# JuliaNeighbors/IVFADC.jl

Hardware: AMD Instinct MI355X
Metric: queries/sec at recall@1 (k=10), SIFT1M-shape d=128 m=8 k=256, 1/2/4/8 GPU (higher is better)
Workload: dtype f32

## Files before the change

include/ivfadc_hip.h:

```cpp
#ifndef IVFADC_HIP_H
#define IVFADC_HIP_H

#include <stddef.h>
#include <stdint.h>

#ifdef __cplusplus
extern "C" {
#endif

typedef struct ivfadc_index ivfadc_t;

typedef enum {
    IVFADC_OK = 0,
    IVFADC_ERR_ASSERT = 1,
    IVFADC_ERR_INVALID = 2,
    IVFADC_ERR_HIP = 3,
    IVFADC_ERR_STATE = 4
} ivfadc_status;

#define IVFADC_ABI_VERSION 4
int ivfadc_abi_version(void);

#define IVFADC_MAX_K 2048
#define IVFADC_MAX_W 2048
// ... 74 lines not shown
int ivfadc_mg_set_gather(ivfadc_mg_t *g, int mode);
int ivfadc_mg_collectives(ivfadc_mg_t *g, int64_t *out);
int ivfadc_mg_append(ivfadc_mg_t *g, int64_t nnew, const float *pts, const uint32_t *ids,
                     int32_t *out_list, uint8_t *out_codes);
int ivfadc_mg_delete_ids(ivfadc_mg_t *g, int64_t ndel, const uint32_t *ids, int64_t *out_removed);
int ivfadc_mg_shift_ids(ivfadc_mg_t *g, int32_t delta);
int ivfadc_mg_search(ivfadc_mg_t *g, int64_t nq, const float *queries, int K, int w,
                     uint32_t *out_ids, float *out_dists, int32_t *out_counts);
void ivfadc_mg_destroy(ivfadc_mg_t *g);

int ivfadc_comm_unique_id(uint8_t *out_id128);
int ivfadc_comm_init(ivfadc_t *h, int nranks, int rank, const uint8_t *id128);
int ivfadc_search_device_allgather(ivfadc_t *h, int64_t nq, const float *d_queries, int K, int w,
                                   int32_t *d_block, int32_t *d_gathered, int slot);
int ivfadc_search_device_allgather_on(ivfadc_t *h, ivfadc_t *searcher, int64_t nq, const float *d_queries, int K, int w,
                                      int32_t *d_block, int32_t *d_gathered, int slot);
int ivfadc_comm_wait(ivfadc_t *h, int64_t *out_collectives);
int ivfadc_comm_destroy(ivfadc_t *h);

int ivfadc_set_list_partition(ivfadc_t *h, int nparts, int part);
int ivfadc_search_device_partial(ivfadc_t *h, int64_t nq, const float *d_queries, int K, int w, uint64_t *d_keys, int32_t *d_counts);
int ivfadc_merge_partials_device(ivfadc_t *h, int64_t nq, int K, int nparts, const uint64_t *d_keys_all, const int32_t *d_counts_all,
                                 uint32_t *d_ids, float *d_dists, int32_t *d_counts);
int64_t ivfadc_listpart_block_words(int64_t nq, int K);
int ivfadc_search_device_listpart(ivfadc_t *h, int64_t nq, const float *d_queries, int K, int w, int32_t *d_block, int32_t *d_gathered,
                                  uint32_t *d_ids, float *d_dists, int32_t *d_counts);

int ivfadc_set_stream(ivfadc_t *h, void *hip_stream);

int ivfadc_ntotal(ivfadc_t *h, int64_t *out_n, int64_t *list_sizes);

int ivfadc_get_lists(ivfadc_t *h, int64_t *offsets, uint8_t *codes, uint32_t *ids);

int ivfadc_get_dims(ivfadc_t *h, int *d, int *kc, int *m, int *ksub);
int ivfadc_get_quantizers(ivfadc_t *h, float *centroids , float *codebooks , uint8_t *code_labels );

int ivfadc_save_index(ivfadc_t *h, const char *path, int index_bits);

int ivfadc_load_index(ivfadc_t **out, int device, const char *path, int *out_index_bits);

int ivfadc_get_rotation(ivfadc_t *h, int *out_rotated, float *out_rot);

typedef struct {
    double   scan_ms;
    double   coarse_ms;
    int64_t  scan_launches;
    int64_t  scanned_points;
    int64_t  queries;
    int32_t  last_qg;
    int32_t  last_chunk;
    int32_t  last_scan_grid;
    int32_t  last_scan_lds;
    int64_t  coarse_fallbacks;
    int32_t  coarse_mfma;
    int32_t  inplace_appends;
    int32_t  last_striped;
    int32_t  coarse_listed;
    int64_t  pruned_points;
    int64_t  lb_survivors;
    int32_t  last_lb;
    int32_t  last_rider;
    double   lb_build_ms;
    int64_t  lb_build_launches;
    int32_t  coarse_prefetched;
    int32_t  last_nf;
    int32_t  last_twolevel;
    int32_t  twolevel_groups;
    int64_t  coarse_visited;
    float    twolevel_probe_fraction;
    int32_t  coarse_f16;
} ivfadc_stats;

int ivfadc_set_profiling(ivfadc_t *h, int on);
int ivfadc_reset_stats(ivfadc_t *h);
int ivfadc_get_stats(ivfadc_t *h, ivfadc_stats *out);

int ivfadc_set_tuning(ivfadc_t *h, int qg, int chunk_points);

int ivfadc_set_coarse_mode(ivfadc_t *h, int mode);

int ivfadc_set_pruning(ivfadc_t *h, int on);

int ivfadc_set_next_queries(ivfadc_t *h, int64_t nq, const float *d_queries, uint64_t token);
int ivfadc_set_query_token(ivfadc_t *h, uint64_t token);

int ivfadc_set_table_mode(ivfadc_t *h, int mode);

int ivfadc_set_u16_tables(ivfadc_t *h, int mode);

int ivfadc_debug_lb_table(ivfadc_t *h, const float *query, int cell, uint8_t *out_table, float *out_consts);

int ivfadc_set_workspace_limit(ivfadc_t *h, uint64_t bytes);

void ivfadc_destroy(ivfadc_t *h);

const char *ivfadc_last_error(void);

#ifdef __cplusplus
}
#endif
#endif
```

ivfadc.jl_amd/_native.py:

```python
import ctypes as C
import os
import subprocess

_HERE = os.path.dirname(os.path.abspath(__file__))
CSRC = os.path.join(_HERE, "csrc")
SO_PATH = os.path.join(CSRC, "libivfadc_hip.so")
SOURCES = [os.path.join(CSRC, "ivfadc_hip.hip"), os.path.join(CSRC, "kernels.hip.h"), os.path.join(CSRC, "train.hip.h"), os.path.join(CSRC, "wave_sort.hip.h"),
           os.path.join(CSRC, "generic.hip.h"), os.path.join(CSRC, "lbscan.hip.h"), os.path.join(CSRC, "nfscan.hip.h"), os.path.join(CSRC, "smallq.hip.h"), os.path.join(CSRC, "twolevel.hip.h"), os.path.join(CSRC, "wg8scan.hip.h"), os.path.join(CSRC, "u16scan.hip.h"),
           os.path.join(os.path.dirname(_HERE), "include", "ivfadc_hip.h")]

HIPCC_FLAGS = ["--offload-arch=gfx950", "-O3", "-ffp-contract=off", "-fno-slp-vectorize", "-fPIC", "-shared", "-std=c++17"]

OK, ERR_ASSERT, ERR_INVALID, ERR_HIP, ERR_STATE = 0, 1, 2, 3, 4


class IVFADCError(RuntimeError):
    def __init__(self, code, msg):
        super().__init__("ivfadc_hip status %d: %s" % (code, msg))
        self.code = code


def needs_build():
    if not os.path.exists(SO_PATH):
        return True
# ... 5 lines not shown
    if not force and not needs_build():
        return SO_PATH
    hipcc = os.environ.get("HIPCC", "/opt/rocm/bin/hipcc")
    cmd = [hipcc] + HIPCC_FLAGS + ["-o", SO_PATH + ".tmp", SOURCES[0]]
    if verbose:
        print(" ".join(cmd))
    subprocess.check_call(cmd, cwd=CSRC)
    os.replace(SO_PATH + ".tmp", SO_PATH)
    return SO_PATH


class Stats(C.Structure):
    _fields_ = [("scan_ms", C.c_double), ("coarse_ms", C.c_double), ("scan_launches", C.c_int64),
                ("scanned_points", C.c_int64), ("queries", C.c_int64), ("last_qg", C.c_int32),
                ("last_chunk", C.c_int32), ("last_scan_grid", C.c_int32), ("last_scan_lds", C.c_int32),
                ("coarse_fallbacks", C.c_int64), ("coarse_mfma", C.c_int32), ("inplace_appends", C.c_int32),
                ("last_striped", C.c_int32), ("coarse_listed", C.c_int32), ("pruned_points", C.c_int64),
                ("lb_survivors", C.c_int64), ("last_lb", C.c_int32), ("last_rider", C.c_int32),
                ("lb_build_ms", C.c_double), ("lb_build_launches", C.c_int64),
                ("coarse_prefetched", C.c_int32), ("last_nf", C.c_int32), ("last_twolevel", C.c_int32), ("twolevel_groups", C.c_int32),
                ("coarse_visited", C.c_int64), ("twolevel_probe_fraction", C.c_float), ("coarse_f16", C.c_int32)]


class HostStats(C.Structure):
    _fields_ = [("stage_in_us", C.c_double), ("enqueue_us", C.c_double), ("wait_us", C.c_double), ("stage_out_us", C.c_double),
                ("calls", C.c_int64), ("batches", C.c_int64), ("queries_direct", C.c_int64), ("results_direct", C.c_int64),
                ("zero_copy", C.c_int64), ("streams_replaced", C.c_int64)]


ABI_VERSION = 4

_lib = None


def lib():
    global _lib
    if _lib is not None:
        return _lib
    if not os.path.exists(SO_PATH):
        raise IVFADCError(ERR_STATE, "libivfadc_hip.so is not built (run __graft_entry__.build()); "
                                     "there is no CPU fallback")
    L = C.CDLL(SO_PATH)
    vp, fp, u8p = C.c_void_p, C.POINTER(C.c_float), C.POINTER(C.c_uint8)
    i32p, u32p, i64p = C.POINTER(C.c_int32), C.POINTER(C.c_uint32), C.POINTER(C.c_int64)
    L.ivfadc_last_error.restype = C.c_char_p
    L.ivfadc_create.argtypes = [C.POINTER(vp), C.c_int, C.c_int, C.c_int, C.c_int, C.c_int, fp, fp, u8p]
    L.ivfadc_set_lists.argtypes = [vp, i64p, u8p, u32p]
    L.ivfadc_create_u16.argtypes = [C.POINTER(vp), C.c_int, C.c_int, C.c_int, C.c_int, C.c_int, fp, fp, vp]
    L.ivfadc_code_bits.argtypes = [vp, C.POINTER(C.c_int)]
    L.ivfadc_set_lists_u16.argtypes = [vp, i64p, vp, u32p]
    L.ivfadc_get_lists_u16.argtypes = [vp, i64p, vp, u32p]
    L.ivfadc_encode_u16.argtypes = [vp, C.c_int64, fp, i32p, vp]
    L.ivfadc_append_u16.argtypes = [vp, C.c_int64, fp, u32p, i32p, vp]
    L.ivfadc_get_quantizers_u16.argtypes = [vp, fp, fp, vp]
    L.ivfadc_train.argtypes = [C.c_int, C.c_int, C.c_int64, fp, C.c_int, C.c_int, C.c_int, C.c_int, C.c_int, C.c_uint64, fp, fp]
    L.ivfadc_train.restype = C.c_int
    L.ivfadc_synth_lists.argtypes = [vp, i64p, C.c_uint64]
    L.ivfadc_encode.argtypes = [vp, C.c_int64, fp, i32p, u8p]
    L.ivfadc_append.argtypes = [vp, C.c_int64, fp, u32p, i32p, u8p]
    L.ivfadc_search.argtypes = [vp, C.c_int64, fp, C.c_int, C.c_int, u32p, fp, i32p]
    L.ivfadc_debug_lb_table.argtypes = [vp, fp, C.c_int, u8p, fp]
    L.ivfadc_get_dims.argtypes = [vp, i32p, i32p, i32p, i32p]
    L.ivfadc_get_quantizers.argtypes = [vp, fp, fp, u8p]
    L.ivfadc_search_device.argtypes = [vp, C.c_int64, vp, C.c_int, C.c_int, vp, vp, vp]
    L.ivfadc_coarse_search.argtypes = [vp, C.c_int64, fp, C.c_int, i32p, fp]
    L.ivfadc_coarse_search_device.argtypes = [vp, C.c_int64, vp, C.c_int, vp, vp]
    L.ivfadc_search_preassigned.argtypes = [vp, C.c_int64, fp, C.c_int, C.c_int, i32p, fp, u32p, fp, i32p]
    L.ivfadc_search_device_preassigned.argtypes = [vp, C.c_int64, vp, C.c_int, C.c_int, vp, vp, vp, vp, vp]
    for name in ("coarse_search", "coarse_search_device", "search_preassigned", "search_device_preassigned"):
        getattr(L, "ivfadc_" + name).restype = C.c_int
    L.ivfadc_sync.argtypes = [vp]
    L.ivfadc_set_stream.argtypes = [vp, vp]
    L.ivfadc_ntotal.argtypes = [vp, i64p, i64p]
    L.ivfadc_get_lists.argtypes = [vp, i64p, u8p, u32p]
    L.ivfadc_set_profiling.argtypes = [vp, C.c_int]
    L.ivfadc_reset_stats.argtypes = [vp]
    L.ivfadc_get_stats.argtypes = [vp, C.POINTER(Stats)]
    L.ivfadc_set_tuning.argtypes = [vp, C.c_int, C.c_int]
    L.ivfadc_set_workspace_limit.argtypes = [vp, C.c_uint64]
    L.ivfadc_set_coarse_mode.argtypes = [vp, C.c_int]
    L.ivfadc_set_pruning.argtypes = [vp, C.c_int]
    L.ivfadc_set_next_queries.argtypes = [vp, C.c_int64, C.c_void_p, C.c_uint64]
    L.ivfadc_set_query_token.argtypes = [vp, C.c_uint64]
    L.ivfadc_search_batches.argtypes = [vp, C.c_int, i64p, fp, C.c_int, C.c_int, u32p, fp, i32p]
    L.ivfadc_set_table_mode.argtypes = [vp, C.c_int]
    L.ivfadc_set_u16_tables.argtypes = [vp, C.c_int]
    L.ivfadc_set_u16_tables.restype = C.c_int
    L.ivfadc_delete_ids.argtypes = [vp, C.c_int64, u32p, i64p]
    L.ivfadc_shift_ids.argtypes = [vp, C.c_int32]
    L.ivfadc_save_index.argtypes = [vp, C.c_char_p, C.c_int]
    L.ivfadc_load_index.argtypes = [C.POINTER(vp), C.c_int, C.c_char_p, C.POINTER(C.c_int)]
    L.ivfadc_get_rotation.argtypes = [vp, C.POINTER(C.c_int), fp]
    L.ivfadc_destroy.argtypes = [vp]
    L.ivfadc_destroy.restype = None
    L.ivfadc_abi_version.argtypes = []
    L.ivfadc_abi_version.restype = C.c_int
    if L.ivfadc_abi_version() != ABI_VERSION:
        raise IVFADCError(ERR_STATE, "libivfadc_hip.so has ABI version %d, this binding was written for %d: rebuild "
                                     "(__graft_entry__.build())" % (L.ivfadc_abi_version(), ABI_VERSION))
    L.ivfadc_host_alloc.argtypes = [C.c_size_t, C.POINTER(vp)]
    L.ivfadc_host_free.argtypes = [vp]
    L.ivfadc_host_register.argtypes = [vp, C.c_size_t]
    L.ivfadc_host_unregister.argtypes = [vp]
    L.ivfadc_get_host_stats.argtypes = [vp, C.POINTER(HostStats)]
    L.ivfadc_reset_host_stats.argtypes = [vp]
    for name in ("host_alloc", "host_free", "host_register", "host_unregister", "get_host_stats", "reset_host_stats"):
        getattr(L, "ivfadc_" + name).restype = C.c_int
    L.ivfadc_mg_create.argtypes = [C.POINTER(vp), C.c_int, i32p, C.c_int, C.c_int, C.c_int, C.c_int, fp, fp, u8p]
    L.ivfadc_mg_set_lists.argtypes = [vp, i64p, u8p, u32p]
    L.ivfadc_mg_append.argtypes = [vp, C.c_int64, fp, u32p, i32p, u8p]
    L.ivfadc_mg_delete_ids.argtypes = [vp, C.c_int64, u32p, i64p]
    L.ivfadc_mg_shift_ids.argtypes = [vp, C.c_int32]
    L.ivfadc_mg_search.argtypes = [vp, C.c_int64, fp, C.c_int, C.c_int, u32p, fp, i32p]
    L.ivfadc_mg_synth_lists.argtypes = [vp, i64p, C.c_uint64]
    L.ivfadc_mg_num_devices.argtypes = [vp]
    L.ivfadc_mg_set_gather.argtypes = [vp, C.c_int]
    L.ivfadc_mg_collectives.argtypes = [vp, i64p]
    L.ivfadc_comm_unique_id.argtypes = [u8p]
    L.ivfadc_comm_init.argtypes = [vp, C.c_int, C.c_int, u8p]
    L.ivfadc_search_device_allgather.argtypes = [vp, C.c_int64, vp, C.c_int, C.c_int, vp, vp, C.c_int]
    L.ivfadc_search_device_allgather_on.argtypes = [vp, vp, C.c_int64, vp, C.c_int, C.c_int, vp, vp, C.c_int]
    L.ivfadc_clone_view.argtypes = [vp, C.POINTER(vp)]
    L.ivfadc_set_list_partition.argtypes = [vp, C.c_int, C.c_int]
    L.ivfadc_search_device_partial.argtypes = [vp, C.c_int64, vp, C.c_int, C.c_int, vp, vp]
    L.ivfadc_merge_partials_device.argtypes = [vp, C.c_int64, C.c_int, C.c_int, vp, vp, vp, vp, vp]
    L.ivfadc_listpart_block_words.argtypes = [C.c_int64, C.c_int]
    L.ivfadc_listpart_block_words.restype = C.c_int64
    L.ivfadc_search_device_listpart.argtypes = [vp, C.c_int64, vp, C.c_int, C.c_int, vp, vp, vp, vp, vp]
    L.ivfadc_comm_wait.argtypes = [vp, i64p]
    L.ivfadc_comm_destroy.argtypes = [vp]
    L.ivfadc_mg_destroy.argtypes = [vp]
    L.ivfadc_mg_destroy.restype = None
    for name in ("mg_create", "mg_set_lists", "mg_append", "mg_search", "mg_delete_ids", "mg_shift_ids", "mg_synth_lists",
                 "mg_num_devices", "mg_set_gather", "mg_collectives", "set_list_partition", "search_device_partial", "merge_partials_device", "search_device_listpart", "comm_unique_id", "comm_init", "search_device_allgather", "search_device_allgather_on", "clone_view", "comm_wait", "comm_destroy"):
        getattr(L, "ivfadc_" + name).restype = C.c_int
    for name in ("create", "set_lists", "synth_lists", "encode", "append", "search", "search_device", "sync", "set_stream",
                 "ntotal", "get_lists", "set_profiling", "reset_stats", "get_stats", "set_tuning", "set_workspace_limit", "set_coarse_mode", "set_pruning", "set_table_mode", "set_next_queries", "set_query_token", "search_batches", "save_index", "load_index", "delete_ids", "shift_ids"):
        getattr(L, "ivfadc_" + name).restype = C.c_int
    _lib = L
    return L


def check(rc):
    if rc == OK:
        return
    msg = lib().ivfadc_last_error().decode("utf-8", "replace")
    if rc == ERR_ASSERT:
        raise AssertionError(msg)
    raise IVFADCError(rc, msg)


def ptr(a, ty):
    return None if a is None else a.ctypes.data_as(C.POINTER(ty))


class PinnedArray:

    def __init__(self, shape, dtype):
        import numpy as np
        self.shape = tuple(int(x) for x in (shape if isinstance(shape, (tuple, list)) else (shape,)))
        self.dtype = np.dtype(dtype)
        n = int(np.prod(self.shape)) if self.shape else 1
        self.nbytes = max(1, n * self.dtype.itemsize)
        p = C.c_void_p()
        check(lib().ivfadc_host_alloc(self.nbytes, C.byref(p)))
        self._p = p
        buf = (C.c_char * self.nbytes).from_address(p.value)
        self.a = np.frombuffer(buf, dtype=self.dtype, count=n).reshape(self.shape)

    def close(self):
        if self._p is not None and self._p.value:
            self.a = None
            lib().ivfadc_host_free(self._p)
            self._p = None

    def __del__(self):
        try:
            self.close()
        except Exception:
            pass


def host_register(a):
    assert a.flags["C_CONTIGUOUS"]
    check(lib().ivfadc_host_register(C.c_void_p(a.ctypes.data), a.nbytes))


def host_unregister(a):
    check(lib().ivfadc_host_unregister(C.c_void_p(a.ctypes.data)))
```

ivfadc.jl_amd/csrc/ivfadc_hip.hip:

```cpp
#include "../../include/ivfadc_hip.h"
#include "kernels.hip.h"
#include "train.hip.h"
#include "generic.hip.h"
#include "u16scan.hip.h"
#include "twolevel.hip.h"

#include <algorithm>
#include <atomic>
#include <chrono>
#include <cmath>
#include <cstdarg>
#include <cstdio>
#include <cstdlib>
#include <cstring>
#include <mutex>
#include <new>
#include <stdexcept>
#include <string>
#include <thread>
#include <vector>

#include <dlfcn.h>
#include <execinfo.h>
#include <fcntl.h>
// ... 248 lines not shown
    bool allow_nf = true;
    DevBuf wg8_tabs, wg8_items;
    int wg8_mode = 0;
    int u16_tables = 0;
    bool u16_wide = false;
    bool wg8_wide = false;
    int part_n = 1, part_i = 0;
    uint64_t *partial_keys = nullptr;
    int64_t partial_nq = -1;
    int partial_w = 0, partial_K = 0;
    DevBuf sq_keys, sq_cnt, sq_arrive, cent_t;
    bool allow_sq = true, sq_inside = false;
    bool allow_lb = true;
    bool force_lb = false;
    DevBuf cent_hi, cent_lo, q_hi, q_lo;
    DevBuf cent_f16, q_f16, q_flags;
    float f16_scale = 0.f;
    bool allow_f16 = true, last_coarse_f16 = false;
    int dp32 = 0;
    bool allow_bf16 = true, last_coarse_bf16 = false;
    bool allow_prune = true;
    bool allow_listed = true, last_listed = false;
    void *comm = nullptr;
    int comm_ranks = 0, comm_rank = 0;
    hipStream_t comm_stream = nullptr;
    hipEvent_t comm_ready = nullptr;
    static constexpr int COMM_SLOTS = 8;
    hipEvent_t comm_done[COMM_SLOTS] = {};
    bool comm_busy[COMM_SLOTS] = {};
    int64_t comm_collectives = 0;
    int64_t comm_seq = 0, comm_slot_seq[COMM_SLOTS] = {}, comm_waited = 0;
    bool allow_filt = true;
    DevBuf tl_centres, tl_off, tl_rad, tl_cent, tl_slot, tl_gdist;
    int tl_G = 0, tl_mode = 0;
    bool dev_entry = false;
    PinnedBuf fb_pin;
    hipEvent_t fb_ev = nullptr;
    bool fb_pending = false;
    int fb_countdown = 0;
    int64_t fb_sp = 0, fb_pp = 0;
    float prune_est = -1.0f;
    RelaxedInt lane_ticket;
    int my_ticket = -1;
    RelaxedInt n_views;
    bool tl_tried = false, tl_use = false;
    float tl_eps = 0.f, tl_probe_fraction = -1.f;
    int64_t visited_base = 0;
    DevBuf gen_a, gen_b, gen_tmp, gen_off, gen_tot;
    int tlist_ldq = 0;
    int tmin_tiles = 0, tmin_tile_w = 0;
    float cmaxn = 0.f;
    bool allow_mfma = true;
    int mfma_min_kc = 2048;
    int64_t n = 0;
    bool have_lists = false;
    bool synthetic = false;
    bool dirty = false;
    int64_t maxlen = 0;
    int64_t inplace_appends = 0;
    DevBuf list_pos, list_len, list_codeoff, codes, ids, app_stage;
    std::vector<int64_t> h_len;
    std::vector<std::vector<uint8_t>> hl_codes;
    std::vector<std::vector<uint32_t>> hl_ids;
    std::vector<int64_t> d_cap, d_pos, d_codeoff;
    int64_t ntotal() const
    {
        int64_t t = 0;
        for (int64_t v : h_len) t += v;
        return t;
    }
    std::vector<uint8_t> h_label_ok;
    bool identity_labels = false;
    bool u16 = false;
    int cb = 0;
    std::vector<uint16_t> lab16;
    std::vector<uint32_t> lab_sorted;
    std::vector<float> rot;

    const float *hint_q = nullptr, *pf_q = nullptr, *avail_q = nullptr;
    int64_t hint_nq = 0, pf_nq = 0, avail_nq = 0;
    uint64_t hint_token = 0, pf_token = 0, cur_token = 0, own_token = 0;
    hipEvent_t hint_ev = nullptr;
    DevBuf cdist2;
    DevBuf pre_list, pre_dc;
    DevBuf q_stage, cdist, probe_list, probe_dc, probe_base, list_cnt, bucket_off, wi_off, cursor, bucket_items, misc,
        qthr, part_keys, part_cnt, out_ids, out_dists, out_counts, assign, enc_codes, pts_stage, dbg;
    PinnedBuf pin_in, pin_out;
    bool hc_out_direct = false;
    hipStream_t copy_stream = nullptr;
    hipStream_t copy_probed_a = nullptr, copy_probed_b = nullptr;
    std::vector<hipEvent_t> ingest_ev;
    ivfadc_host_stats hstats{};
    int64_t carry_queries = 0, carry_scanned = 0, carry_pruned = 0, carry_surv = 0, carry_fallbacks = 0, carry_launches = 0;
    size_t qthr_armed = 0;
    bool list_cnt_armed = false;
    size_t ws_budget = (size_t)8 << 30;

    bool profiling = false;
    int profiling_level = 0;
    struct EvPair { hipEvent_t a, b; int kind; };
    std::vector<EvPair> pending;
    std::vector<EvPair> free_ev;
    ivfadc_stats stats{};
    int64_t scanned_base = 0, fallback_base = 0, pruned_base = 0, surv_base = 0;
    int force_qg = 0, force_chunk = 0;
    bool own_stream = true;
    struct FnCfg { const void *fn; size_t lds; int occ; };
    std::vector<FnCfg> fn_cfg;

    ivfadc_index *view_of = nullptr;
    bool is_view = false, orphan = false;
    uint64_t generation = 0, view_gen = 0;
    std::vector<ivfadc_index *> views;
    ivfadc_index *pipe_view = nullptr;
    hipEvent_t pipe_ev_in = nullptr;
};

struct HandleLock {
    ivfadc_index *h;
    explicit HandleLock(ivfadc_index *x) : h(x)
    {
        if (!h) return;
        if (h->is_view) {
            std::lock_guard<std::recursive_mutex> topo(g_topo_mu);
            h->mu.m.lock();
        } else {
            h->mu.m.lock();
        }
    }
    ~HandleLock() { if (h) h->mu.m.unlock(); }
    HandleLock(const HandleLock &) = delete;
    HandleLock &operator=(const HandleLock &) = delete;
};

namespace {

int wait_stream(ivfadc_index *h)
{
    for (int i = 0; i < 200000; ++i) {
        const hipError_t e = hipStreamQuery(h->stream);
        if (e == hipSuccess) return IVFADC_OK;
        if (e != hipErrorNotReady) return fail(IVFADC_ERR_HIP, "hipStreamQuery failed: %s", hipGetErrorString(e));
        if (i > 20000) break;
    }
    HIP_TRY(hipStreamSynchronize(h->stream));
    return IVFADC_OK;
}

int set_device(ivfadc_index *h)
{
    HIP_TRY(hipSetDevice(h->device));
    return IVFADC_OK;
}

int ev_begin(ivfadc_index *h, int kind, ivfadc_index::EvPair &ep)
{
    if (!h->free_ev.empty()) {
        ep = h->free_ev.back();
        h->free_ev.pop_back();
    } else {
        HIP_TRY(hipEventCreate(&ep.a));
        HIP_TRY(hipEventCreate(&ep.b));
    }
    ep.kind = kind;
    HIP_TRY(hipEventRecord(ep.a, h->stream));
    return IVFADC_OK;
// ... 644 lines not shown
        e->max_lds = lds;
    }
    return IVFADC_OK;
}

int fn_occupancy(ivfadc_index *h, const void *fn, size_t lds, int &occ, bool abs_lds = true, int threads = 256)
{
    TRY(fn_raise_lds(h->device, fn, lds, abs_lds));
    occ = 0;
    for (auto &c : h->fn_cfg)
        if (c.fn == fn && c.lds == lds) occ = c.occ;
    if (occ == 0) {
        HIP_TRY(hipOccupancyMaxActiveBlocksPerMultiprocessor(&occ, fn, threads, lds));
        occ = std::max(1, std::min(occ, 8));
        h->fn_cfg.push_back({fn, lds, occ});
    }
    return IVFADC_OK;
}

int run_twolevel(ivfadc_index *h, const float *d_q, int64_t nb, int w, int *d_probe_list, float *d_probe_dc, u32 *d_probe_base, u32 *d_list_cnt,
                 u64 *d_scanned)
{
    const int G = h->tl_G;
    TRY(h->tl_gdist.ensure((size_t)nb * G * 4));
    ivfadc_index::EvPair ep;
    if (h->profiling) TRY(ev_begin(h, 1, ep));
    launch_coarse_exact(h, d_q, nb, h->tl_centres.as<float>(), G, h->tl_gdist.as<float>(), false);
    HIP_TRY(hipGetLastError());
    TwoLevelView tv;
    tv.gdist = h->tl_gdist.as<float>();
    tv.g_off = h->tl_off.as<u32>();
    tv.g_rad = h->tl_rad.as<float>();
    tv.cent_g = h->tl_cent.as<float>();
    tv.slot_id = h->tl_slot.as<u32>();
    tv.G = G;
    tv.d = h->d;
    tv.eps = h->tl_eps;
    const size_t lds = (size_t)4 * h->d * 4 + 4 * 64 * 8;
    if (lds > (size_t)(48 << 10)) TRY(fn_raise_lds(h->device, (const void *)twolevel_topw_kernel, lds, false));
    hipLaunchKernelGGL(twolevel_topw_kernel, dim3((unsigned)((nb + 3) / 4)), dim3(256), lds, h->stream, d_q, tv, (int)nb, w, h->list_len.as<u32>(),
                       d_probe_list, d_probe_dc, d_probe_base, d_list_cnt, d_scanned, h->part_n, h->part_i);
    HIP_TRY(hipGetLastError());
    if (h->profiling) TRY(ev_end(h, ep));
    return IVFADC_OK;
}

int launch_topw(ivfadc_index *h, const float *d_q, int64_t n, int w, int capw, bool mfma, bool wpq4, int *out_list, float *out_dc, u32 *out_base,
                u32 *lc, u64 *counters, int part_n, int part_i)
{
    const size_t lds = (size_t)4 * capw * 8;
    void (*fn)(const float *, int, int, int, int, const u32 *, int *, float *, u32 *, u32 *, u64 *, const RefineArgs, int, int);
    if (mfma)
        fn = wpq4 ? topw_select_kernel<true, 4, true> : topw_select_kernel<true, 1, true>;
    else if (w <= 64)
        fn = wpq4 ? topw_select_kernel<true, 4, false> : topw_select_kernel<true, 1, false>;
    else
        fn = wpq4 ? topw_select_kernel<false, 4, false> : topw_select_kernel<false, 1, false>;
    const unsigned grid = wpq4 ? (unsigned)n : (unsigned)((n + 3) / 4);
    if (lds > (size_t)(32 << 10)) { int occ_unused = 0; TRY(fn_occupancy(h, (const void *)fn, lds, occ_unused, false)); }
    hipLaunchKernelGGL(fn, dim3(grid), dim3(256), lds, h->stream, h->cdist.as<float>(), (int)n, h->kc, w, capw, h->list_len.as<u32>(), out_list,
                       out_dc, out_base, lc, counters, refine_args(h, d_q), part_n, part_i);
    HIP_TRY(hipGetLastError());
    return IVFADC_OK;
}

LbView lb_view(const ivfadc_index *h)
{
    LbView v;
    v.cb_split = h->lb_split.as<uint4>();
    v.cb_n2 = h->lb_n2.as<float>();
    v.cb_lab = h->lb_lab.as<float>();
    v.cb_maxn = h->lb_maxn.as<float>();
    v.cb_f16 = (h->lb_use_f16 && h->lb_f16.p) ? h->lb_f16.as<uint4>() : (const uint4 *)nullptr;
    v.cb_isc = h->lb_isc.as<float>();
    v.mu = v.cb_f16 ? 1.48e-3f : 9.2e-5f;
    return v;
}

int probe_stage(ivfadc_index *h, const Plan &pl, int64_t nb, const float *d_q, int w, bool single, u32 *lc, const int *pre_list, const float *pre_dc)
{
    const bool pre = pre_list != nullptr;
    u64 *d_scanned = h->misc.as<u64>();
    const bool wpq4 = !pl.lanes && nb * 1 < (int64_t)8 * h->num_cu * 4 && h->kc >= 512 && !(pl.form == ScanForm::QueryMajorLb && !pl.fuse_topw);
    const bool have_rows = single && !pre && !pl.coarse_mfma && !pl.twolevel && h->avail_q == d_q && h->avail_nq == nb && h->cdist2.p != nullptr;
    h->avail_q = nullptr;
    if (pre || pl.twolevel || have_rows) {
        h->tmin_tiles = 0;
        h->last_listed = false;
    }
    if (pre) {
        hipLaunchKernelGGL(probe_ingest_kernel, dim3((unsigned)((nb + 3) / 4)), dim3(256), 0, h->stream, pre_list, pre_dc, (int)nb, h->kc, w,
                           h->list_len.as<u32>(), h->probe_list.as<int>(), h->probe_dc.as<float>(), h->probe_base.as<u32>(), lc, (u32 *)nullptr,
                           d_scanned);
        HIP_TRY(hipGetLastError());
    } else if (pl.twolevel) {
        TRY(run_twolevel(h, d_q, nb, w, h->probe_list.as<int>(), h->probe_dc.as<float>(), h->probe_base.as<u32>(), lc, d_scanned));
    } else if (have_rows) {
        std::swap(h->cdist, h->cdist2);
    } else {
        TRY(run_coarse(h, d_q, nb, pl.coarse_mfma, pl.coarse_mfma && (pl.fuse_topw ? h->m > 16 : !wpq4),
                       !pl.fuse_topw && !wpq4, w));
    }
    if (!pl.fuse_topw && !pl.twolevel && !pre)
        TRY(launch_topw(h, d_q, nb, w, pl.capw, pl.coarse_mfma, wpq4, h->probe_list.as<int>(), h->probe_dc.as<float>(), h->probe_base.as<u32>(), lc,
                        d_scanned, h->part_n, h->part_i));
    h->stats.last_rider = 0;
    h->stats.coarse_prefetched = have_rows ? 1 : 0;
    h->stats.last_twolevel = pl.twolevel ? 1 : 0;
    h->stats.coarse_mfma = pl.coarse_mfma ? 1 : 0;
    h->stats.coarse_f16 = (pl.coarse_mfma && h->last_coarse_f16 && !have_rows) ? 1 : 0;
    h->stats.coarse_listed = h->last_listed ? 1 : 0;
    return IVFADC_OK;
}

int scan_query_major(ivfadc_index *h, const Plan &pl, int64_t nb, const float *d_q, int K, int w, uint32_t *d_ids, float *d_dists, int32_t *d_counts,
                     bool single, bool pre)
{
    const int kc = h->kc;
    const bool lb = pl.form == ScanForm::QueryMajorLb;
    QScanArgs a;
    a.ix = index_view(h);
    a.queries = d_q;
    a.nq = (int)nb; a.w = w; a.K = K; a.cap = pl.cap;
    a.probe_list = h->probe_list.as<int>(); a.probe_dc = h->probe_dc.as<float>(); a.probe_base = h->probe_base.as<u32>();
    a.out_ids = d_ids; a.out_dists = d_dists; a.out_counts = d_counts;
    a.cdist = pl.fuse_topw ? h->cdist.as<float>() : (const float *)nullptr;
    a.scanned_points = h->misc.as<u64>();
    a.approx = pl.coarse_mfma ? 1 : 0;
    a.rf = refine_args(h, d_q);
    a.prune = h->allow_prune ? (pre ? 2 : 1) : 0;
    a.lb = lb_view(h);
    int occ = 0;
    TRY(fn_occupancy(h, pl.fn, pl.lds, occ));
    ivfadc_index::EvPair ep;
    const bool ride = single && !pre && !h->tl_use && h->hint_q != nullptr && h->hint_nq > 0 && !lb && pl.small_k && (h->d & 7) == 0 &&
                      (!h->allow_mfma || kc < h->mfma_min_kc) && (h->hint_nq + 4 * RIDER_QW - 1) / (4 * RIDER_QW) <= 65535 &&
                      (size_t)h->hint_nq * kc * 4 <= h->ws_budget / 4;
    qscan_coarse_fn_t fk = ride ? pick_qscan_coarse(h->m, h->dsub, pl.qg) : nullptr;
    if (fk) {
        TRY(h->cdist2.ensure((size_t)h->hint_nq * kc * 4));
        CoarseNext cn;
        cn.queries = h->hint_q; cn.out = h->cdist2.as<float>(); cn.nq = (int)h->hint_nq; cn.ncx = (kc + 63) / 64;
        const size_t lds = std::max<size_t>(pl.lds, (size_t)64 * 132 * 4);
        TRY(fn_raise_lds(h->device, (const void *)fk, lds, true));
        const unsigned grid = (unsigned)(nb + (int64_t)cn.ncx * ((h->hint_nq + 4 * RIDER_QW - 1) / (4 * RIDER_QW)));
        if (h->hint_ev) {
            HIP_TRY(hipStreamWaitEvent(h->stream, h->hint_ev, 0));
            h->hint_ev = nullptr;
        }
        if (h->profiling) TRY(ev_begin(h, 0, ep));
        hipLaunchKernelGGL(fk, dim3(grid), dim3(256), lds, h->stream, a, cn);
        HIP_TRY(hipGetLastError());
        if (h->profiling) TRY(ev_end(h, ep));
        h->pf_q = h->hint_q;
        h->pf_nq = h->hint_nq;
        h->pf_token = h->hint_token;
        h->stats.last_rider = 1;
    } else {
        if (h->profiling) TRY(ev_begin(h, 0, ep));
        hipLaunchKernelGGL((qscan_fn_t)pl.fn, dim3((unsigned)nb), dim3(pl.threads), pl.lds, h->stream, a);
        HIP_TRY(hipGetLastError());
        if (h->profiling) TRY(ev_end(h, ep));
    }
    h->stats.last_scan_grid = (int)nb;
    if (!lb) TRY(fb_snapshot(h));
    if (h->profiling_level >= 2 && lb && !pl.fuse_topw && pl.qg == 4) {
        void (*bk)(const IndexView, const LbView, const float *, const int *, int, u32 *) =
            (h->m == 48) ? lb_build_only_kernel<48, 16, 4> : lb_build_only_kernel<16, 6, 4>;
        TRY(fn_raise_lds(h->device, (const void *)bk, pl.lds, false));
        TRY(h->dbg.ensure((size_t)nb * 4));
        ivfadc_index::EvPair eb;
        TRY(ev_begin(h, 2, eb));
        hipLaunchKernelGGL(bk, dim3((unsigned)nb), dim3(256), pl.lds, h->stream, a.ix, a.lb, d_q, h->probe_list.as<int>(), w,
                           h->dbg.as<u32>());
        HIP_TRY(hipGetLastError());
        TRY(ev_end(h, eb));
    }
    return IVFADC_OK;
}

template <class... P, class... X>
int launch_list_scan(ivfadc_index *h, const Plan &pl, size_t upper, void (*fn)(const ScanArgs, P...), const ScanArgs &a, X... extra)
{
    int occ = 0;
    TRY(fn_occupancy(h, pl.fn, pl.lds, occ, true, pl.threads));
    const unsigned grid = (unsigned)std::max<size_t>(1, std::min<size_t>(upper, (size_t)h->num_cu * occ));
    ivfadc_index::EvPair ep;
    if (h->profiling) TRY(ev_begin(h, 0, ep));
    hipLaunchKernelGGL(fn, dim3(grid), dim3(pl.threads), pl.lds, h->stream, a, extra...);
    HIP_TRY(hipGetLastError());
    if (h->profiling) TRY(ev_end(h, ep));
    h->stats.last_scan_grid = (int)grid;
    return IVFADC_OK;
}

int scan_list_major(ivfadc_index *h, const Plan &pl, int64_t nb, const float *d_q, int K, int w, uint32_t *d_ids, float *d_dists, int32_t *d_counts,
                    bool direct)
{
    const int kc = h->kc;
    const size_t np = (size_t)nb * w;
    const bool w8 = pl.form == ScanForm::EightWave;
    u32 *d_qhead = (u32 *)((char *)h->misc.p + 4096);
    TRY(h->bucket_items.ensure(np * 4));
    TRY(h->part_keys.ensure(np * pl.maxch * K * 8));
    TRY(h->part_cnt.ensure(np * pl.maxch * 4));
    {
        const size_t before = h->qthr.bytes;
        TRY(h->qthr.ensure((size_t)nb * 8));
        if (h->qthr.bytes != before) h->qthr_armed = 0;
        if (h->qthr_armed < (size_t)nb) {
            const size_t cnt = h->qthr.bytes / 8;
            hipLaunchKernelGGL(fill_u64_kernel, dim3(256), dim3(256), 0, h->stream, h->qthr.as<u64>(), cnt, (u64)KEY_MAX);
            HIP_TRY(hipGetLastError());
            h->qthr_armed = cnt;
        }
    }
    if (!direct) {
        u32 *item_list = nullptr;
        if (w8) {
            TRY(h->wg8_items.ensure(np * (size_t)pl.maxch * 4));
            item_list = h->wg8_items.as<u32>();
        }
        hipLaunchKernelGGL(bucket_scan_kernel, dim3(1), dim3(1024), 0, h->stream, h->list_cnt.as<u32>(), h->list_len.as<u32>(),
                           kc, pl.qg, pl.CH, h->bucket_off.as<u32>(), h->wi_off.as<u32>(), h->cursor.as<u32>(), d_qhead, item_list);
        HIP_TRY(hipGetLastError());
        hipLaunchKernelGGL(bucket_scatter_kernel, dim3((unsigned)((np + 255) / 256)), dim3(256), 0, h->stream,
                           h->probe_list.as<int>(), (int)np, h->bucket_off.as<u32>(), h->cursor.as<u32>(), h->bucket_items.as<u32>(),
                           h->part_n, h->part_i);
        HIP_TRY(hipGetLastError());
    }

    ScanArgs a;
    a.ix = index_view(h);
    a.queries = d_q;
    a.w = w; a.K = K; a.cap = pl.cap;
    a.probe_dc = h->probe_dc.as<float>(); a.probe_base = h->probe_base.as<u32>(); a.list_cnt = h->list_cnt.as<u32>();
    a.bucket_off = h->bucket_off.as<u32>(); a.wi_off = h->wi_off.as<u32>(); a.bucket_items = h->bucket_items.as<u32>();
    a.queue_head = d_qhead;
    a.qthr = h->qthr.as<u64>();
    a.part_keys = h->part_keys.as<u64>(); a.part_cnt = h->part_cnt.as<u32>(); a.maxch = pl.maxch; a.CH = pl.CH;
// ... 94 lines not shown

int check_view_current(ivfadc_index *h)
{
    if (!h->is_view) return IVFADC_OK;
    if (h->orphan || !h->view_of) return fail(IVFADC_ERR_STATE, "the index this view was taken from has been destroyed");
    if (h->view_of->generation != h->view_gen) return fail(IVFADC_ERR_STATE, "the index has changed since this view was taken: take a new one");
    return IVFADC_OK;
}

int check_search_args(ivfadc_index *h, int64_t nq, int K, int &w)
{
    if (!h) return fail(IVFADC_ERR_INVALID, "null handle");
    TRY(check_view_current(h));
    if (K < 1) return fail(IVFADC_ERR_ASSERT, "Number of neighbors must be k >= 1");
    if (w < 1) return fail(IVFADC_ERR_ASSERT, "Number of clusters to search in must be w >= 1");
    if (nq < 0) return fail(IVFADC_ERR_INVALID, "nq < 0");
    if (!h->have_lists && !h->dirty) return fail(IVFADC_ERR_STATE, "no inverted lists set");
    w = std::min(w, h->kc);
    if ((int64_t)nq * K > ((int64_t)1 << 40)) return fail(IVFADC_ERR_INVALID, "nq x K = %lld result slots", (long long)nq * K);
    return IVFADC_OK;
}

int gen_sort(ivfadc_index *h, const u64 *in, u64 *out, int64_t total, int segments, const u32 *d_off)
{
    if (total == 0) return IVFADC_OK;
    size_t tmp = 0;
    HIP_TRY(rocprim::segmented_radix_sort_keys(nullptr, tmp, in, out, (unsigned)total, (unsigned)segments, d_off, d_off + 1, 0, 64,
                                               h->stream));
    TRY(h->gen_tmp.ensure(std::max<size_t>(tmp, 16)));
    HIP_TRY(rocprim::segmented_radix_sort_keys(h->gen_tmp.p, tmp, in, out, (unsigned)total, (unsigned)segments, d_off, d_off + 1, 0, 64,
                                               h->stream));
    return IVFADC_OK;
}

int gen_stage_a(ivfadc_index *h, const float *qa, int64_t na, int w, int *d_pl, float *d_pd, u32 *d_pb, u64 *d_scanned)
{
    const int kc = h->kc;
    TRY(run_coarse(h, qa, na, false));
    const int64_t rk = na * kc;
    TRY(h->gen_a.ensure((size_t)rk * 8));
    TRY(h->gen_b.ensure((size_t)rk * 8));
    hipLaunchKernelGGL(gen_row_keys_kernel, dim3((unsigned)std::min<int64_t>(8192, (rk + 255) / 256)), dim3(256), 0, h->stream,
                       h->cdist.as<float>(), rk, kc, h->gen_a.as<u64>());
    HIP_TRY(hipGetLastError());
    std::vector<u32> off((size_t)na + 1);
    for (int64_t q = 0; q <= na; ++q) off[q] = (u32)(q * kc);
    TRY(h->gen_off.ensure(((size_t)na + 1) * 4));
    TRY(h2d_copy(h->gen_off.p, off.data(), ((size_t)na + 1) * 4, h->stream));
    HIP_TRY(hipStreamSynchronize(h->stream));
    TRY(gen_sort(h, h->gen_a.as<u64>(), h->gen_b.as<u64>(), rk, (int)na, h->gen_off.as<u32>()));
    hipLaunchKernelGGL(gen_probes_kernel, dim3((unsigned)na), dim3(256), 0, h->stream, h->gen_b.as<u64>(), kc, w, h->list_len.as<u32>(),
                       d_pl, d_pd, d_pb, h->gen_tot.as<u32>(), d_scanned);
    HIP_TRY(hipGetLastError());
    return IVFADC_OK;
}

int search_generic(ivfadc_index *h, int64_t nq, const float *d_q, int K, int w, uint32_t *d_ids, float *d_dists, int32_t *d_counts,
                   const int *pre_list = nullptr, const float *pre_dc = nullptr)
{
    const int kc = h->kc;
    const size_t lds = (align_up((size_t)h->d, 4) + (h->u16 ? (size_t)GEN16_TILE : (size_t)h->m * 256)) * 4;
    if (lds > LDS_MAX) return fail(IVFADC_ERR_INVALID, "m=%d needs %zu B of LDS in the generic path (> %zu)", h->m, lds, LDS_MAX);
    void (*dump)(const IndexView, const float *, int, const int *, const float *, const u32 *, const u32 *, u64 *) =
        h->u16 ? gen_dump_u16_kernel : gen_dump_kernel;
    TRY(fn_raise_lds(h->device, (const void *)dump, lds, false));
    TRY(ensure_common_ws(h));
    u64 *d_scanned = h->misc.as<u64>();
    const IndexView ix = index_view(h);
    const u32 *idp = h->synthetic ? (const u32 *)nullptr : h->ids.as<u32>();
    const int64_t per_q = (int64_t)kc * (4 + 16) + (int64_t)w * 12 + 64;
    int64_t nba = std::max<int64_t>(1, (int64_t)(h->ws_budget / (size_t)per_q));
    nba = std::min<int64_t>(std::min<int64_t>(nba, nq), std::min<int64_t>(65535, ((int64_t)1 << 31) / std::max(1, kc)));
    std::vector<u32> tot, off;
    for (int64_t a0 = 0; a0 < nq; a0 += nba) {
        const int64_t na = std::min(nba, nq - a0);
        const float *qa = d_q + (size_t)a0 * h->d;
        const size_t np = (size_t)na * w;
        TRY(h->probe_list.ensure(np * 4));
        TRY(h->probe_dc.ensure(np * 4));
        TRY(h->probe_base.ensure(np * 4));
        TRY(h->gen_tot.ensure((size_t)na * 4));
        if (pre_list) {
            hipLaunchKernelGGL(probe_ingest_kernel, dim3((unsigned)((na + 3) / 4)), dim3(256), 0, h->stream, pre_list + (size_t)a0 * w,
                               pre_dc + (size_t)a0 * w, (int)na, kc, w, h->list_len.as<u32>(), h->probe_list.as<int>(), h->probe_dc.as<float>(),
                               h->probe_base.as<u32>(), (u32 *)nullptr, h->gen_tot.as<u32>(), d_scanned);
            HIP_TRY(hipGetLastError());
        } else {
            TRY(gen_stage_a(h, qa, na, w, h->probe_list.as<int>(), h->probe_dc.as<float>(), h->probe_base.as<u32>(), d_scanned));
        }
        tot.resize((size_t)na);
        TRY(d2h_copy(tot.data(), h->gen_tot.p, (size_t)na * 4, h->stream));
        HIP_TRY(hipStreamSynchronize(h->stream));
        const int64_t cap_keys = std::max<int64_t>(1 << 20, (int64_t)(h->ws_budget / 24));
        for (int64_t g0 = 0; g0 < na;) {
            int64_t g1 = g0, keys = 0;
            while (g1 < na && (g1 == g0 || keys + tot[g1] <= cap_keys) && keys + tot[g1] < ((int64_t)1 << 32)) keys += tot[g1++];
            if (g1 == g0) return fail(IVFADC_ERR_INVALID, "a single query probes %u points: too many for one sort", tot[g0]);
            const int64_t ng = g1 - g0;
            off.resize((size_t)ng + 1);
            off[0] = 0;
            for (int64_t q = 0; q < ng; ++q) off[q + 1] = off[q] + tot[g0 + q];
            TRY(h->gen_a.ensure((size_t)std::max<int64_t>(1, keys) * 8));
            TRY(h->gen_b.ensure((size_t)std::max<int64_t>(1, keys) * 8));
            TRY(h->gen_off.ensure(((size_t)ng + 1) * 4));
            TRY(h2d_copy(h->gen_off.p, off.data(), ((size_t)ng + 1) * 4, h->stream));
            const int *pl = h->probe_list.as<int>() + (size_t)g0 * w;
            const float *pd = h->probe_dc.as<float>() + (size_t)g0 * w;
            const u32 *pb = h->probe_base.as<u32>() + (size_t)g0 * w;
            for (int64_t y0 = 0; y0 < ng; y0 += 32768) {
                const int64_t ny = std::min<int64_t>(32768, ng - y0);
                hipLaunchKernelGGL(dump, dim3((unsigned)w, (unsigned)ny), dim3(256), lds, h->stream, ix,
                                   qa + (size_t)(g0 + y0) * h->d, w, pl + (size_t)y0 * w, pd + (size_t)y0 * w, pb + (size_t)y0 * w,
                                   h->gen_off.as<u32>() + y0, h->gen_a.as<u64>());
                HIP_TRY(hipGetLastError());
            }
            TRY(gen_sort(h, h->gen_a.as<u64>(), h->gen_b.as<u64>(), keys, (int)ng, h->gen_off.as<u32>()));
            hipLaunchKernelGGL(gen_emit_kernel, dim3((unsigned)ng), dim3(256), 0, h->stream, h->gen_b.as<u64>(), h->gen_off.as<u32>(),
                               h->gen_tot.as<u32>() + g0, w, K, pl, pb, h->list_pos.as<int64_t>(), idp, d_ids + (size_t)(a0 + g0) * K,
                               d_dists + (size_t)(a0 + g0) * K, d_counts + a0 + g0);
            HIP_TRY(hipGetLastError());
            HIP_TRY(hipStreamSynchronize(h->stream));
            g0 = g1;
        }
        h->stats.queries += na;
    }
    h->stats.last_qg = -2;
    h->stats.coarse_mfma = 0;
    return IVFADC_OK;
}

int sq_inside_kc(const ivfadc_index *h)
{
    return (h->sq_inside && h->cent_t.p) ? SQ_COARSE_INSIDE : 0;
}

bool sq_eligible(const ivfadc_index *h, int64_t nq, int K, int w)
{
    static const bool off = getenv("IVFADC_NO_SMALLQ") != nullptr;
    if (off || !h->allow_sq || h->force_qg != 0 || h->u16) return false;
    if (K > 64 || w > 64 || nq > 64 || nq * w > 512) return false;
    if ((h->d & 3) != 0) return false;
    const size_t lds = scan_lds_bytes(h, 1, 64, true) + 64 + (h->kc <= sq_inside_kc(h) ? (size_t)h->kc * 4 : 0);
    return lds <= LDS_MAX;
}

int search_small(ivfadc_index *h, int64_t nq, const float *d_q, int K, int w, uint32_t *d_ids, float *d_dists, int32_t *d_counts)
{
    TRY(ensure_common_ws(h));
    const bool inside = h->kc <= sq_inside_kc(h);
    if (!inside) {
        if (h->cent_t.p && nq <= 65535) {
            TRY(h->cdist.ensure((size_t)nq * h->kc * 4));
            ivfadc_index::EvPair ec;
            if (h->profiling) TRY(ev_begin(h, 1, ec));
            void (*ck)(const float4 *, const float *, float *, int, int, int) =
                h->d == 128 ? coarse_lane_kernel<32> : (h->d == 96 ? coarse_lane_kernel<24> : (h->d == 64 ? coarse_lane_kernel<16> : coarse_lane_kernel<0>));
            hipLaunchKernelGGL(ck, dim3((unsigned)((h->kc + 255) / 256), (unsigned)nq), dim3(256), 0, h->stream,
                               h->cent_t.as<float4>(), d_q, h->cdist.as<float>(), (int)nq, h->kc, h->d);
            HIP_TRY(hipGetLastError());
            if (h->profiling) TRY(ev_end(h, ec));
        } else {
            TRY(run_coarse(h, d_q, nq, false));
        }
    }
    const int64_t items = nq * w;
    int nch = (int)std::max<int64_t>(1, std::min<int64_t>((h->maxlen + 4095) / 4096, (2 * (int64_t)h->num_cu) / std::max<int64_t>(1, items)));
    uint32_t CH = (uint32_t)align_up((size_t)std::max<int64_t>(1, (h->maxlen + nch - 1) / nch), 1024);
// ... 124 lines not shown
            any = true;
        }
        if (!any) break;
    }
    mem.erase(std::remove_if(mem.begin(), mem.end(), [](const std::vector<int> &l) { return l.empty(); }), mem.end());
    const int G2 = (int)mem.size();
    std::vector<float> gc((size_t)G2 * d);
    std::vector<u32> off((size_t)G2 + 1, 0);
    for (int g = 0; g < G2; ++g) {
        std::vector<float> c_;
        centre_of(mem[g], c_);
        std::copy(c_.begin(), c_.end(), gc.begin() + (size_t)g * d);
        off[g + 1] = off[g] + (u32)mem[g].size();
    }
    const size_t slots = off[G2];
    std::vector<u32> slot_id(std::max<size_t>(slots, 1), 0xFFFFFFFFu);
    std::vector<float> grouped(std::max<size_t>(slots, 1) * d, 0.0f), rad((size_t)G2, 0.0f);
    for (int g = 0; g < G2; ++g) {
        const u32 ns = off[g + 1] - off[g];
        float *blk = grouped.data() + (size_t)off[g] * d;
        double r2max = 0.0;
        for (u32 sl = 0; sl < ns; ++sl) {
            const int c = mem[g][sl];
            slot_id[off[g] + sl] = (u32)c;
            for (int i = 0; i < d; ++i) blk[((size_t)(i >> 2) * ns + sl) * 4 + (i & 3)] = cent[(size_t)c * d + i];
            r2max = std::max(r2max, dist2(c, &gc[(size_t)g * d]));
        }
        rad[g] = std::nextafter((float)(std::sqrt(r2max) * (1.0 + 1e-6)), INFINITY);
    }
    TRY(h->tl_centres.ensure(gc.size() * 4));
    TRY(h->tl_off.ensure(off.size() * 4));
    TRY(h->tl_rad.ensure(rad.size() * 4));
    TRY(h->tl_cent.ensure(grouped.size() * 4 + 64));
    TRY(h->tl_slot.ensure(slot_id.size() * 4));
    TRY(h2d_copy(h->tl_centres.p, gc.data(), gc.size() * 4, h->stream));
    TRY(h2d_copy(h->tl_off.p, off.data(), off.size() * 4, h->stream));
    TRY(h2d_copy(h->tl_rad.p, rad.data(), rad.size() * 4, h->stream));
    TRY(h2d_copy(h->tl_cent.p, grouped.data(), grouped.size() * 4, h->stream));
    TRY(h2d_copy(h->tl_slot.p, slot_id.data(), slot_id.size() * 4, h->stream));
    G = G2;
    h->tl_G = G;
    h->tl_eps = (float)(d + 16) * 1.1920929e-7f;
    {
        const int64_t ns = std::min<int64_t>(1024, kc);
        const int wp = std::min(32, kc);
        TRY(ensure_common_ws(h));
        DevBuf pl_, pd_, pb_;
        int rc = pl_.ensure((size_t)ns * wp * 4);
        if (rc == IVFADC_OK) rc = pd_.ensure((size_t)ns * wp * 4);
        if (rc == IVFADC_OK) rc = pb_.ensure((size_t)ns * wp * 4);
        u64 before[512], after[512];
        if (rc == IVFADC_OK) {
            HIP_TRY(hipStreamSynchronize(h->stream));
            HIP_TRY(hipMemcpy(before, h->misc.p, sizeof(before), hipMemcpyDeviceToHost));
            const bool prof = h->profiling;
            h->profiling = false;
            rc = run_twolevel(h, h->centroids.as<float>(), ns, wp, pl_.as<int>(), pd_.as<float>(), pb_.as<u32>(), nullptr, h->misc.as<u64>());
            h->profiling = prof;
        }
        if (rc == IVFADC_OK) {
            HIP_TRY(hipStreamSynchronize(h->stream));
            HIP_TRY(hipMemcpy(after, h->misc.p, sizeof(after), hipMemcpyDeviceToHost));
            u64 vis = 0;
            for (int i = 0; i < 64; ++i) vis += after[i * 8 + 3] - before[i * 8 + 3];
            HIP_TRY(h2d_hip(h->misc.p, before, sizeof(before), h->stream));
            h->tl_probe_fraction = (float)((double)vis / ((double)ns * (double)kc));
        }
        pl_.release(); pd_.release(); pb_.release();
        if (rc != IVFADC_OK) return rc;
    }
    h->tl_use = h->tl_mode > 0 || (h->tl_mode == 0 && h->tl_probe_fraction >= 0.f && h->tl_probe_fraction <= TL_AUTO_MAX_FRACTION);
    return IVFADC_OK;
}

struct PreProbes { const int *lists; const float *dcs; };

int search_dev(ivfadc_index *h, int64_t nq, const float *d_q, int K, int w, uint32_t *d_ids, float *d_dists, int32_t *d_counts,
               const PreProbes *pre = nullptr)
{
    HintScope hint_scope{h};
    const bool declared = h->cur_token != 0 && h->cur_token == h->pf_token;
    h->avail_q = declared ? h->pf_q : nullptr;
    h->avail_nq = declared ? h->pf_nq : 0;
    h->pf_q = nullptr; h->pf_nq = 0; h->pf_token = 0; h->cur_token = 0;
    h->stats.coarse_prefetched = 0;
    h->stats.last_rider = 0;
    h->partial_nq = -1;
    TRY(set_device(h));
    if (h->dirty) TRY(upload_lists(h));
    if (nq == 0) return IVFADC_OK;
    if (!pre && !h->tl_tried && !h->is_view && h->tl_mode >= 0 && (h->tl_mode > 0 || h->kc >= TL_AUTO_MIN_KC)) TRY(build_twolevel(h));
    const bool parted = h->part_n > 1;
    const int *prl = pre ? pre->lists : (const int *)nullptr;
    const float *prd = pre ? pre->dcs : (const float *)nullptr;
    if (!parted && !pre && sq_eligible(h, nq, K, w)) return search_small(h, nq, d_q, K, w, d_ids, d_dists, d_counts);
    if (K > IVFADC_MAX_K || w > IVFADC_MAX_W || h->force_qg == -2 || (h->u16 && K > 64 && !h->u16_wide)) {
        if (parted) return fail(IVFADC_ERR_INVALID, "list-partitioned mode reaches K <= %d and w <= %d", IVFADC_MAX_K, IVFADC_MAX_W);
        return search_generic(h, nq, d_q, K, w, d_ids, d_dists, d_counts, prl, prd);
    }
    Plan pl;
    TRY(fb_poll(h));
    TRY(h->u16 ? make_plan_u16(h, nq, K, w, pl, pre != nullptr) : make_plan(h, nq, K, w, pl, pre != nullptr));
    if (!pl.fits) {
        if (parted) return fail(IVFADC_ERR_INVALID, "list-partitioned mode: the selection kernels' LDS need exceeds a CU for this m and K");
        return search_generic(h, nq, d_q, K, w, d_ids, d_dists, d_counts, prl, prd);
    }
    if (parted && pl.nb < nq)
        return fail(IVFADC_ERR_INVALID, "list-partitioned mode: the batch must fit one sub-batch (raise ivfadc_set_workspace_limit or split the batch)");
    for (int64_t b0 = 0; b0 < nq; b0 += pl.nb) {
        const int64_t nb = std::min(pl.nb, nq - b0);
        TRY(search_subbatch(h, pl, nb, d_q + (size_t)b0 * h->d, K, w, d_ids + (size_t)b0 * K, d_dists + (size_t)b0 * K,
                            d_counts + b0, pl.nb >= nq, pre ? prl + (size_t)b0 * w : prl, pre ? prd + (size_t)b0 * w : prd));
    }
    return IVFADC_OK;
}

int coarse_dev(ivfadc_index *h, int64_t nq, const float *d_q, int w, int32_t *d_lists, float *d_dists)
{
    HintScope hint_scope{h};
    h->pf_q = nullptr; h->pf_nq = 0; h->pf_token = 0; h->cur_token = 0;
    h->stats.coarse_prefetched = 0;
    h->stats.last_rider = 0;
    h->partial_nq = -1;
    TRY(set_device(h));
    if (h->dirty) TRY(upload_lists(h));
    if (nq == 0) return IVFADC_OK;
    if (!h->tl_tried && !h->is_view && h->tl_mode >= 0 && (h->tl_mode > 0 || h->kc >= TL_AUTO_MIN_KC)) TRY(build_twolevel(h));
    TRY(ensure_common_ws(h));
    const int kc = h->kc;
    u64 *d_sink = (u64 *)((char *)h->misc.p + MISC_SINK);
    const bool generic = w > IVFADC_MAX_W;
    const CoarseForm cf = coarse_form(h, w, !generic, true);
    const bool twolevel = cf.twolevel, mfma = cf.mfma;
    const size_t per_q = (twolevel ? (size_t)h->tl_G : (size_t)kc) * (generic ? 20 : 4) + (size_t)w * 4 + 64;
    int64_t nb = (int64_t)std::max<size_t>(generic ? 1 : 64, h->ws_budget / per_q);
    nb = std::min<int64_t>(nb, (int64_t)1 << 22);
    if (twolevel) nb = std::min<int64_t>(nb, std::max<int64_t>(1, ((int64_t)1 << 30) / std::max(1, h->tl_G)));
    if (generic) nb = std::min<int64_t>(nb, std::min<int64_t>(65535, ((int64_t)1 << 31) / std::max(1, kc)));
    nb = std::max<int64_t>(1, std::min<int64_t>(nb, nq));
    TRY(h->probe_base.ensure((size_t)nb * w * 4));
    h->stats.last_twolevel = twolevel ? 1 : 0;
    h->stats.coarse_mfma = mfma ? 1 : 0;
    for (int64_t b0 = 0; b0 < nq; b0 += nb) {
        const int64_t n = std::min(nb, nq - b0);
        const float *q = d_q + (size_t)b0 * h->d;
        int *ol = (int *)d_lists + (size_t)b0 * w;
        float *od = d_dists + (size_t)b0 * w;
        if (generic) {
            TRY(h->gen_tot.ensure((size_t)n * 4));
            TRY(gen_stage_a(h, q, n, w, ol, od, h->probe_base.as<u32>(), d_sink));
            continue;
        }
        if (twolevel) {
            TRY(run_twolevel(h, q, n, w, ol, od, h->probe_base.as<u32>(), nullptr, d_sink));
            h->tmin_tiles = 0;
            h->last_listed = false;
            continue;
        }
        const bool wpq4 = n < (int64_t)8 * h->num_cu * 4 && kc >= 512;
        TRY(run_coarse(h, q, n, mfma, mfma && !wpq4, !wpq4, w));
        TRY(launch_topw(h, q, n, w, sel_cap(w), mfma, wpq4, ol, od, h->probe_base.as<u32>(), nullptr, d_sink, 1, 0));
        h->stats.coarse_f16 = (mfma && h->last_coarse_f16) ? 1 : 0;
        h->stats.coarse_listed = h->last_listed ? 1 : 0;
    }
    return IVFADC_OK;
}

int encode_dev(ivfadc_index *h, int64_t n, const float *pts, int32_t *out_list, uint8_t *out_codes)
{
    const int64_t bmax = std::max<int64_t>(256, (int64_t)(((size_t)1 << 30) / ((size_t)h->kc * 4)));
    const size_t lds = align_up((size_t)h->d, 4) * 4 + (size_t)h->m * 8;
    for (int64_t b0 = 0; b0 < n; b0 += bmax) {
        const int64_t nb = std::min(bmax, n - b0);
        TRY(h->pts_stage.ensure((size_t)nb * h->d * 4));
        TRY(h->assign.ensure((size_t)nb * 4));
        TRY(h->enc_codes.ensure((size_t)nb * h->cb));
        TRY(h2d_copy(h->pts_stage.p, pts + (size_t)b0 * h->d, (size_t)nb * h->d * 4, h->stream));
        TRY(run_coarse(h, h->pts_stage.as<float>(), nb, false));
        hipLaunchKernelGGL(argmin_rows_kernel, dim3((unsigned)((nb + 3) / 4)), dim3(256), 0, h->stream, h->cdist.as<float>(), (int)nb,
                           h->kc, h->assign.as<int>());
        HIP_TRY(hipGetLastError());
        if (h->u16)
            hipLaunchKernelGGL(encode_u16_kernel, dim3((unsigned)nb), dim3(256), lds, h->stream, h->pts_stage.as<float>(), h->assign.as<int>(),
                               h->d, h->m, h->ksub, h->dsub, h->centroids.as<float>(), h->codebooks.as<float>(), h->enc_codes.as<uint16_t>());
        else
        hipLaunchKernelGGL(encode_kernel, dim3((unsigned)nb), dim3(256), lds, h->stream, h->pts_stage.as<float>(), h->assign.as<int>(),
                           h->d, h->m, h->ksub, h->dsub, h->centroids.as<float>(), h->codebooks.as<float>(), h->labels.as<uint8_t>(),
                           h->enc_codes.as<uint8_t>());
        HIP_TRY(hipGetLastError());
        TRY(d2h_copy(out_list + b0, h->assign.p, (size_t)nb * 4, h->stream));
        TRY(d2h_copy(out_codes + (size_t)b0 * h->cb, h->enc_codes.p, (size_t)nb * h->cb, h->stream));
        HIP_TRY(hipStreamSynchronize(h->stream));
    }
    return IVFADC_OK;
}

}

namespace {

struct TrainCtx {
    hipStream_t stream = nullptr;
    DevBuf cdist, assign, mind, partial, acc, counts, flag, blockmax;
};

// ... 427 lines not shown
                        }
                    }
                }
            }
            if (rc == IVFADC_OK) rc = h->cent_hi.ensure(hi.size() * 2);
            if (rc == IVFADC_OK) rc = h->cent_lo.ensure(lo.size() * 2);
            if (rc == IVFADC_OK) {
                e = h2d_hip(h->cent_hi.p, hi.data(), hi.size() * 2, h->stream);
                if (e == hipSuccess) e = h2d_hip(h->cent_lo.p, lo.data(), lo.size() * 2, h->stream);
                if (e != hipSuccess) rc = fail(IVFADC_ERR_HIP, "upload failed: %s", hipGetErrorString(e));
            }
        } else {
            h->allow_bf16 = false;
        }
        if (getenv("IVFADC_NO_PRUNE") != nullptr) h->allow_prune = false;
        if (rc == IVFADC_OK) rc = h->cnorm.ensure((size_t)kc * 4);
        if (rc == IVFADC_OK) {
            e = h2d_hip(h->cnorm.p, cn.data(), (size_t)kc * 4, h->stream);
            if (e != hipSuccess) rc = fail(IVFADC_ERR_HIP, "upload failed: %s", hipGetErrorString(e));
        }
        h->allow_filt = getenv("IVFADC_EXACT_TABLES") == nullptr;
        h->allow_mfma = getenv("IVFADC_COARSE_EXACT") == nullptr;
    }
    if (rc != IVFADC_OK) { ivfadc_destroy(h); return rc; }
    h->h_len.assign((size_t)kc, 0);
    h->hl_codes.assign((size_t)kc, {});
    h->hl_ids.assign((size_t)kc, {});
    h->dirty = true;
    *out = h;
    return IVFADC_OK;
}

int ivfadc_create(ivfadc_t **out, int device, int d, int kc, int m, int ksub, const float *centroids, const float *codebooks,
                  const uint8_t *code_labels)
try {
    return create_impl(out, device, d, kc, m, ksub, centroids, codebooks, code_labels, nullptr);
} IVF_CATCH

int ivfadc_create_u16(ivfadc_t **out, int device, int d, int kc, int m, int ksub, const float *centroids, const float *codebooks,
                      const void *code_labels)
try {
    if (!code_labels) {
        if (out) *out = nullptr;
        return fail(IVFADC_ERR_INVALID, "null array");
    }
    return create_impl(out, device, d, kc, m, ksub, centroids, codebooks, nullptr, (const uint16_t *)code_labels);
} IVF_CATCH

int ivfadc_code_bits(ivfadc_t *h, int *bits)
try {
    HandleLock lk_(h);
    if (!h || !bits) return fail(IVFADC_ERR_INVALID, "null argument");
    *bits = h->u16 ? 16 : 8;
    return IVFADC_OK;
} IVF_CATCH

void ivfadc_destroy(ivfadc_t *h)
{
    if (!h) return;
    std::unique_lock<std::recursive_mutex> topo(g_topo_mu);
    h->mu.m.lock();
    h->mu.m.unlock();
    (void)hipSetDevice(h->device);
    if (h->pipe_view) { ivfadc_destroy(h->pipe_view); h->pipe_view = nullptr; }
    if (h->fb_ev) { (void)hipEventSynchronize(h->fb_ev); (void)hipEventDestroy(h->fb_ev); }
    h->fb_pin.release();
    if (h->pipe_ev_in) (void)hipEventDestroy(h->pipe_ev_in);
    if (h->copy_stream) { (void)hipStreamSynchronize(h->copy_stream); (void)hipStreamDestroy(h->copy_stream); }
    for (hipEvent_t e : h->ingest_ev) (void)hipEventDestroy(e);
    for (ivfadc_index *v : h->views) {
        std::lock_guard<std::recursive_mutex> vl(v->mu.m);
        v->orphan = true;
        v->view_of = nullptr;
    }
    if (h->is_view && h->view_of) {
        auto &vs = h->view_of->views;
        vs.erase(std::remove(vs.begin(), vs.end(), h), vs.end());
        h->view_of->n_views.store((int)vs.size());
    }
    if (h->stream) (void)hipStreamSynchronize(h->stream);
    if (h->comm || h->comm_stream) (void)ivfadc_comm_destroy(h);
    for (auto &ep : h->pending) { (void)hipEventDestroy(ep.a); (void)hipEventDestroy(ep.b); }
    for (auto &ep : h->free_ev) { (void)hipEventDestroy(ep.a); (void)hipEventDestroy(ep.b); }
    DevBuf *bufs[] = {&h->lb_f16, &h->lb_isc, &h->cent_f16, &h->q_f16, &h->q_flags, &h->tl_centres, &h->tl_off, &h->tl_rad, &h->tl_cent, &h->tl_slot, &h->tl_gdist, &h->cdist2, &h->pre_list, &h->pre_dc, &h->cent_t, &h->sq_keys, &h->sq_cnt, &h->sq_arrive, &h->lb_split, &h->lb_n2, &h->lb_lab, &h->lb_maxn, &h->nf_n2, &h->nf_lab, &h->wg8_tabs, &h->wg8_items, &h->centroids, &h->codebooks, &h->codebooks_t, &h->codebooks_p, &h->labels, &h->cnorm, &h->tmin, &h->tlist, &h->cent_hi, &h->cent_lo, &h->q_hi, &h->q_lo, &h->gen_a, &h->gen_b, &h->gen_tmp, &h->gen_off, &h->gen_tot, &h->list_pos, &h->list_len, &h->list_codeoff, &h->codes, &h->ids, &h->app_stage, &h->q_stage,
                      &h->cdist, &h->probe_list, &h->probe_dc, &h->probe_base, &h->list_cnt, &h->bucket_off, &h->wi_off, &h->cursor,
                      &h->bucket_items, &h->misc, &h->qthr, &h->part_keys, &h->part_cnt, &h->out_ids, &h->out_dists, &h->out_counts,
                      &h->assign, &h->enc_codes, &h->pts_stage, &h->dbg};
    for (DevBuf *b : bufs) b->release();
    h->pin_in.release();
    h->pin_out.release();
    if (h->stream && h->own_stream) (void)hipStreamDestroy(h->stream);
    delete h;
}

static int streams_serialised(hipStream_t a, hipStream_t b, bool &serial)
{
    serial = false;
    double best = 1e30;
    for (int rep = 0; rep < 2; ++rep) {
        HIP_TRY(hipStreamSynchronize(a));
        HIP_TRY(hipStreamSynchronize(b));
        const auto t0 = std::chrono::steady_clock::now();
        hipLaunchKernelGGL(spin_us_kernel, dim3(1), dim3(64), 0, a, 60u);
        hipLaunchKernelGGL(spin_us_kernel, dim3(1), dim3(64), 0, b, 60u);
        HIP_TRY(hipGetLastError());
        HIP_TRY(hipStreamSynchronize(a));
        HIP_TRY(hipStreamSynchronize(b));
        best = std::min(best, std::chrono::duration<double, std::micro>(std::chrono::steady_clock::now() - t0).count());
    }
    serial = best > 105.0;
    return IVFADC_OK;
}

static int ensure_overlap(const hipStream_t *fixed, int nfixed, hipStream_t *cand, int64_t *replaced)
{
    static const bool off = getenv("IVFADC_NO_STREAM_PROBE") != nullptr;
    if (off) return IVFADC_OK;
    std::vector<hipStream_t> rejected;
    int rc = IVFADC_OK;
    for (int attempt = 0; attempt < 6; ++attempt) {
        bool clash = false;
        for (int i = 0; i < nfixed && !clash && rc == IVFADC_OK; ++i) {
            if (!fixed[i] || fixed[i] == *cand) continue;
            rc = streams_serialised(fixed[i], *cand, clash);
        }
        if (rc != IVFADC_OK || !clash) break;
        hipStream_t next = nullptr;
        if (hipStreamCreateWithFlags(&next, hipStreamNonBlocking) != hipSuccess) { (void)hipGetLastError(); break; }
        rejected.push_back(*cand);
        *cand = next;
        if (replaced) ++*replaced;
    }
    for (hipStream_t s : rejected) (void)hipStreamDestroy(s);
    return rc;
}

static int clone_view(ivfadc_index *src, ivfadc_index **out)
{
    *out = nullptr;
    if (src->is_view) return fail(IVFADC_ERR_STATE, "a view of a view: take it from the index itself");
    TRY(set_device(src));
    if (src->dirty) TRY(upload_lists(src));
    if (!src->have_lists) return fail(IVFADC_ERR_STATE, "no inverted lists set");
    HIP_TRY(hipStreamSynchronize(src->stream));
    std::vector<std::vector<uint8_t>> keep_codes;
    std::vector<std::vector<uint32_t>> keep_ids;
    keep_codes.swap(src->hl_codes);
    keep_ids.swap(src->hl_ids);
    ivfadc_index *v = nullptr;
    try { v = new ivfadc_index(*src); } catch (...) { keep_codes.swap(src->hl_codes); keep_ids.swap(src->hl_ids); throw; }
    keep_codes.swap(src->hl_codes);
    keep_ids.swap(src->hl_ids);
    DevBuf *shared[] = {&v->lb_f16, &v->lb_isc, &v->cent_f16, &v->tl_centres, &v->tl_off, &v->tl_rad, &v->tl_cent, &v->tl_slot, &v->centroids, &v->codebooks, &v->codebooks_t, &v->codebooks_p, &v->labels, &v->cnorm, &v->lb_split, &v->lb_n2, &v->lb_lab,
                        &v->lb_maxn, &v->nf_n2, &v->nf_lab, &v->cent_t, &v->cent_hi, &v->cent_lo, &v->list_pos, &v->list_len, &v->list_codeoff,
                        &v->codes, &v->ids};
    for (DevBuf *b : shared) b->alias();
    DevBuf *scratch[] = {&v->wg8_tabs, &v->wg8_items, &v->q_f16, &v->q_flags, &v->tl_gdist, &v->cdist2, &v->pre_list, &v->pre_dc, &v->sq_keys, &v->sq_cnt, &v->sq_arrive, &v->tmin, &v->tlist, &v->q_hi, &v->q_lo, &v->gen_a, &v->gen_b, &v->gen_tmp,
                         &v->gen_off, &v->gen_tot, &v->app_stage, &v->q_stage, &v->cdist, &v->probe_list, &v->probe_dc, &v->probe_base, &v->list_cnt,
                         &v->bucket_off, &v->wi_off, &v->cursor, &v->bucket_items, &v->misc, &v->qthr, &v->part_keys, &v->part_cnt, &v->out_ids,
                         &v->out_dists, &v->out_counts, &v->assign, &v->enc_codes, &v->pts_stage, &v->dbg};
    for (DevBuf *b : scratch) b->forget();
    v->pin_in.forget();
    v->pin_out.forget();
    v->pending.clear();
    v->free_ev.clear();
    v->views.clear();
    v->n_views.store(0);
    v->my_ticket = -1;
    v->fb_pin.forget();
    v->fb_ev = nullptr;
    v->fb_pending = false;
    v->fb_countdown = 0;
    v->fb_sp = v->fb_pp = 0;
    v->pipe_view = nullptr;
    v->pipe_ev_in = nullptr;
    v->copy_stream = nullptr;
    v->copy_probed_a = v->copy_probed_b = nullptr;
    v->ingest_ev.clear();
    v->hstats = ivfadc_host_stats{};
    v->carry_queries = v->carry_scanned = v->carry_pruned = v->carry_surv = v->carry_fallbacks = v->carry_launches = 0;
    v->comm = nullptr;
    v->comm_stream = nullptr;
    v->comm_ready = nullptr;
    for (int i = 0; i < ivfadc_index::COMM_SLOTS; ++i) { v->comm_done[i] = nullptr; v->comm_busy[i] = false; }
    v->comm_ranks = 0;
    v->comm_rank = 0;
    v->comm_collectives = 0;
    v->comm_seq = 0;
    v->comm_waited = 0;
    for (int i = 0; i < ivfadc_index::COMM_SLOTS; ++i) v->comm_slot_seq[i] = 0;
    v->hint_ev = nullptr;
    v->hint_q = v->pf_q = v->avail_q = nullptr;
    v->hint_nq = v->pf_nq = v->avail_nq = 0;
    v->hint_token = v->pf_token = v->cur_token = 0;
    v->partial_keys = nullptr;
    v->partial_nq = -1;
    v->qthr_armed = 0;
    v->list_cnt_armed = false;
    v->profiling = false;
    v->profiling_level = 0;
    v->stats = ivfadc_stats{};
    v->scanned_base = v->fallback_base = v->pruned_base = v->surv_base = 0;
    v->visited_base = 0;
    v->inplace_appends = 0;
    v->stream = nullptr;
    v->own_stream = true;
    v->is_view = true;
    v->view_of = src;
    v->view_gen = src->generation;
    const hipError_t e = hipStreamCreateWithFlags(&v->stream, hipStreamNonBlocking);
    if (e != hipSuccess) {
        delete v;
        return fail(IVFADC_ERR_HIP, "hipStreamCreateWithFlags failed: %s", hipGetErrorString(e));
    }
    {
        const hipStream_t fixed[1] = {src->stream};
        const int rc = ensure_overlap(fixed, 1, &v->stream, &src->hstats.streams_replaced);
        if (rc != IVFADC_OK) { (void)hipStreamDestroy(v->stream); delete v; return rc; }
    }
    {
        std::lock_guard<std::recursive_mutex> topo(g_topo_mu);
        src->views.push_back(v);
        src->n_views.fetch_add(1);
    }
    *out = v;
    return IVFADC_OK;
}

static void copy_search_config(ivfadc_index *dst, const ivfadc_index *src)
{
    dst->wg8_mode = src->wg8_mode; dst->wg8_wide = src->wg8_wide; dst->u16_wide = src->u16_wide; dst->u16_tables = src->u16_tables;
    dst->allow_nf = src->allow_nf; dst->allow_sq = src->allow_sq; dst->sq_inside = src->sq_inside; dst->allow_lb = src->allow_lb;
    dst->force_lb = src->force_lb; dst->allow_bf16 = src->allow_bf16; dst->allow_f16 = src->allow_f16; dst->lb_use_f16 = src->lb_use_f16; dst->allow_prune = src->allow_prune; dst->allow_listed = src->allow_listed;
    dst->allow_filt = src->allow_filt; dst->allow_mfma = src->allow_mfma; dst->mfma_min_kc = src->mfma_min_kc; dst->ws_budget = src->ws_budget;
    dst->force_qg = src->force_qg; dst->force_chunk = src->force_chunk;
    dst->part_n = src->part_n; dst->part_i = src->part_i;
    dst->tl_use = src->tl_use && dst->tl_cent.p != nullptr; dst->tl_mode = src->tl_mode;
}

int ivfadc_clone_view(ivfadc_t *h, ivfadc_t **out)
try {
    HandleLock lk_(h);
    if (!h || !out) return fail(IVFADC_ERR_INVALID, "null argument");
    return clone_view(h, out);
} IVF_CATCH

static int check_width(ivfadc_index *h, bool want_u16, const char *what)
{
    if (h->u16 && !want_u16) return fail(IVFADC_ERR_STATE, "%s: this index has UInt16 codes; use %s_u16", what, what);
    if (!h->u16 && want_u16) return fail(IVFADC_ERR_STATE, "%s: this index has UInt8 codes; use the entry without _u16", what);
    return IVFADC_OK;
}

static int check_offsets(ivfadc_index *h, const int64_t *offsets, const void *codes, const uint32_t *ids)
{
    const int kc = h->kc;
    if (offsets[0] != 0) return fail(IVFADC_ERR_INVALID, "offsets[0] must be 0");
    for (int l = 0; l < kc; ++l)
        if (offsets[l + 1] < offsets[l]) return fail(IVFADC_ERR_INVALID, "offsets must be non-decreasing (list %d)", l);
    const int64_t n = offsets[kc];
    if (n > (int64_t)0xFFFFFFFFll) return fail(IVFADC_ERR_ASSERT, "index capacity of UInt32 ids exceeded");
    if (n > 0 && (!codes || !ids)) return fail(IVFADC_ERR_INVALID, "null codes/ids");
    return IVFADC_OK;
}

static int set_lists_mirror(ivfadc_t *h, const int64_t *offsets, const uint8_t *codes, const uint32_t *ids, const char *what)
{
    const int kc = h->kc, cb = h->cb;
    TRY(set_device(h));
    MutationScope ms;
    TRY(ms.begin(h, what));
    for (int l = 0; l < kc; ++l) {
        const int64_t a = offsets[l], b = offsets[l + 1];
        h->h_len[l] = b - a;
        h->hl_codes[l].assign(codes + (size_t)a * cb, codes + (size_t)b * cb);
        h->hl_ids[l].assign(ids + a, ids + b);
    }
    return upload_lists(h);
}

static int labels_to_indices(const ivfadc_index *h, int64_t n, const uint16_t *lab, std::vector<uint8_t> &out)
{
    const int m = h->m;
    out.resize((size_t)n * h->cb);
    uint16_t *dst = (uint16_t *)out.data();
    for (int64_t p = 0; p < n; ++p)
        for (int i = 0; i < m; ++i) {
            const uint16_t v = lab[(size_t)p * m + i];
            const int32_t c = h->identity_labels ? (v < h->ksub ? (int32_t)v : -1) : find_label16(h->lab_sorted, h->ksub, i, v);
            if (c < 0) return fail(IVFADC_ERR_INVALID, "code %d of point %lld is not a label of codebook %d", (int)v, (long long)p, i);
            dst[(size_t)p * m + i] = (uint16_t)c;
        }
    return IVFADC_OK;
}

static void indices_to_labels(const ivfadc_index *h, int64_t n, uint16_t *codes)
{
    if (h->identity_labels) return;
    const int m = h->m, ksub = h->ksub;
    for (int64_t p = 0; p < n; ++p)
        for (int i = 0; i < m; ++i) codes[(size_t)p * m + i] = h->lab16[(size_t)i * ksub + codes[(size_t)p * m + i]];
}

int ivfadc_set_lists_u16(ivfadc_t *h, const int64_t *offsets, const void *codes, const uint32_t *ids)
try {
    HandleLock lk_(h);
    if (!h || !offsets) return fail(IVFADC_ERR_INVALID, "null argument");
    TRY(check_width(h, true, "ivfadc_set_lists"));
    TRY(check_mutable(h, "ivfadc_set_lists_u16"));
    TRY(check_offsets(h, offsets, codes, ids));
    std::vector<uint8_t> idx;
    TRY(labels_to_indices(h, offsets[h->kc], (const uint16_t *)codes, idx));
    return set_lists_mirror(h, offsets, idx.data(), ids, "ivfadc_set_lists_u16");
} IVF_CATCH

int ivfadc_set_lists(ivfadc_t *h, const int64_t *offsets, const uint8_t *codes, const uint32_t *ids)
try {
// ... 1478 lines not shown
        for (int i = 0; i < 64; ++i) pp += shards[i * 8 + 1];
        for (int i = 0; i < 64; ++i) sv += shards[i * 8 + 2];
        for (int i = 0; i < 64; ++i) vis += shards[i * 8 + 3];
        HIP_TRY(hipMemcpy(&h->fallback_base, (char *)h->misc.p + 4096 + 64, 8, hipMemcpyDeviceToHost));
    }
    h->scanned_base = sp;
    h->pruned_base = pp;
    h->surv_base = sv;
    h->visited_base = vis;
    const int qg = h->stats.last_qg, ch = h->stats.last_chunk, gr = h->stats.last_scan_grid, lds = h->stats.last_scan_lds;
    const int cm = h->stats.coarse_mfma, ls = h->stats.last_striped, cl = h->stats.coarse_listed, llb = h->stats.last_lb, lnf = h->stats.last_nf;
    const int ltl = h->stats.last_twolevel, lf16 = h->stats.coarse_f16;
    h->stats = ivfadc_stats{};
    h->stats.last_twolevel = ltl;
    h->stats.coarse_f16 = lf16;
    h->stats.last_lb = llb;
    h->stats.last_nf = lnf;
    h->stats.coarse_mfma = cm;
    h->stats.last_striped = ls;
    h->stats.coarse_listed = cl;
    h->stats.last_qg = qg; h->stats.last_chunk = ch; h->stats.last_scan_grid = gr; h->stats.last_scan_lds = lds;
    h->carry_queries = h->carry_scanned = h->carry_pruned = h->carry_surv = h->carry_fallbacks = h->carry_launches = 0;
    if (h->pipe_view) TRY(ivfadc_reset_stats(h->pipe_view));
    return IVFADC_OK;
} IVF_CATCH

int ivfadc_get_stats(ivfadc_t *h, ivfadc_stats *out)
try {
    HandleLock lk_(h);
    if (!h || !out) return fail(IVFADC_ERR_INVALID, "null argument");
    TRY(set_device(h));
    TRY(ev_fold(h));
    HIP_TRY(hipStreamSynchronize(h->stream));
    int64_t sp = 0, pp = 0, sv = 0, vis = 0;
    if (h->misc.p) {
        int64_t shards[512];
        HIP_TRY(hipMemcpy(shards, h->misc.p, sizeof(shards), hipMemcpyDeviceToHost));
        for (int i = 0; i < 64; ++i) sp += shards[i * 8];
        for (int i = 0; i < 64; ++i) pp += shards[i * 8 + 1];
        for (int i = 0; i < 64; ++i) sv += shards[i * 8 + 2];
        for (int i = 0; i < 64; ++i) vis += shards[i * 8 + 3];
        int64_t fb = 0;
        HIP_TRY(hipMemcpy(&fb, (char *)h->misc.p + 4096 + 64, 8, hipMemcpyDeviceToHost));
        h->stats.coarse_fallbacks = fb - h->fallback_base;
    }
    h->stats.scanned_points = sp - h->scanned_base;
    h->stats.pruned_points = pp - h->pruned_base;
    h->stats.lb_survivors = sv - h->surv_base;
    h->stats.coarse_visited = vis - h->visited_base;
    h->stats.twolevel_groups = h->tl_use ? h->tl_G : 0;
    h->stats.twolevel_probe_fraction = h->tl_probe_fraction;
    h->stats.inplace_appends = (int32_t)std::min<int64_t>(h->inplace_appends, 0x7fffffff);
    *out = h->stats;
    out->queries += h->carry_queries;
    out->scanned_points += h->carry_scanned;
    out->pruned_points += h->carry_pruned;
    out->lb_survivors += h->carry_surv;
    out->coarse_fallbacks += h->carry_fallbacks;
    out->scan_launches += h->carry_launches;
    if (h->pipe_view) {
        ivfadc_stats v;
        TRY(ivfadc_get_stats(h->pipe_view, &v));
        out->queries += v.queries;
        out->scanned_points += v.scanned_points;
        out->pruned_points += v.pruned_points;
        out->lb_survivors += v.lb_survivors;
        out->coarse_fallbacks += v.coarse_fallbacks;
        out->scan_launches += v.scan_launches;
        out->coarse_visited += v.coarse_visited;
    }
    return IVFADC_OK;
} IVF_CATCH

int ivfadc_train(int device, int d, int64_t n, const float *data, int kc, int k, int m, int coarse_maxiter, int quant_maxiter,
                 uint64_t seed, float *out_centroids, float *out_codebooks)
try {
    return train_impl(device, d, n, data, kc, k, m, coarse_maxiter, quant_maxiter, seed, out_centroids, out_codebooks);
} IVF_CATCH

int ivfadc_set_coarse_mode(ivfadc_t *h, int mode)
try {
    HandleLock lk_(h);
    if (!h) return fail(IVFADC_ERR_INVALID, "null handle");
    if (mode < 0 || mode > 8) return fail(IVFADC_ERR_INVALID, "mode must be 0 ... 8");
    h->allow_f16 = mode != 8 && mode != 3;
    h->tl_mode = mode == 6 ? 1 : (mode == 7 ? -1 : 0);
    if (h->tl_tried) h->tl_use = h->tl_G > 0 && (h->tl_mode > 0 || (h->tl_mode == 0 && h->tl_probe_fraction >= 0.f && h->tl_probe_fraction <= 0.02f));
    if (h->tl_mode > 0 && h->tl_G == 0) h->tl_tried = false;
    h->sq_inside = mode == 5;
    h->allow_mfma = (mode != 1) && getenv("IVFADC_COARSE_EXACT") == nullptr;
    h->mfma_min_kc = (mode == 2) ? 128 : 2048;
    h->allow_bf16 = mode != 3 && h->cent_hi.p != nullptr;
    h->allow_listed = mode != 4;
    return IVFADC_OK;
} IVF_CATCH

int ivfadc_set_pruning(ivfadc_t *h, int on)
try {
    HandleLock lk_(h);
    if (!h) return fail(IVFADC_ERR_INVALID, "null handle");
    h->allow_prune = on != 0 && getenv("IVFADC_NO_PRUNE") == nullptr;
    return IVFADC_OK;
} IVF_CATCH

int ivfadc_set_next_queries(ivfadc_t *h, int64_t nq, const float *d_queries, uint64_t token)
try {
    HandleLock lk_(h);
    if (!h) return fail(IVFADC_ERR_INVALID, "null handle");
    if (nq < 0) return fail(IVFADC_ERR_INVALID, "nq < 0");
    h->hint_q = (nq > 0 && token != 0) ? d_queries : nullptr;
    h->hint_nq = h->hint_q ? nq : 0;
    h->hint_token = h->hint_q ? token : 0;
    return IVFADC_OK;
} IVF_CATCH

int ivfadc_set_query_token(ivfadc_t *h, uint64_t token)
try {
    HandleLock lk_(h);
    if (!h) return fail(IVFADC_ERR_INVALID, "null handle");
    h->cur_token = token;
    return IVFADC_OK;
} IVF_CATCH

int ivfadc_set_table_mode(ivfadc_t *h, int mode)
try {
    HandleLock lk_(h);
    if (!h) return fail(IVFADC_ERR_INVALID, "null handle");
    if (mode < 0 || mode > 10) return fail(IVFADC_ERR_INVALID, "mode must be 0 ... 10");
    h->allow_filt = mode != 1 && getenv("IVFADC_EXACT_TABLES") == nullptr;
    h->force_lb = mode == 2 || mode == 4;
    h->lb_use_f16 = mode != 3 && mode != 4;
    h->wg8_mode = mode == 5 ? -1 : (mode == 6 || mode == 8 ? 1 : (mode == 7 || mode == 9 ? 2 : 0));
    h->wg8_wide = mode == 8 || mode == 9;
    h->u16_wide = mode == 10;
    return IVFADC_OK;
} IVF_CATCH

int ivfadc_set_u16_tables(ivfadc_t *h, int mode)
try {
    HandleLock lk_(h);
    if (!h) return fail(IVFADC_ERR_INVALID, "null handle");
    if (mode < 0 || mode > 2) return fail(IVFADC_ERR_INVALID, "mode must be 0 ... 2");
    h->u16_tables = mode;
    return IVFADC_OK;
} IVF_CATCH

int ivfadc_debug_lb_table(ivfadc_t *h, const float *query, int cell, uint8_t *out_table, float *out_consts)
try {
    HandleLock lk_(h);
    if (!h || !query || !out_table || !out_consts) return fail(IVFADC_ERR_INVALID, "null argument");
    if (cell < 0 || cell >= h->kc) return fail(IVFADC_ERR_INVALID, "cell out of range");
    if (h->u16) return fail(IVFADC_ERR_STATE, "ivfadc_debug_lb_table: this index has UInt16 codes (no 8-bit lower-bound tables)");
    if (!h->lb_split.p || !lb_shape(h->m, h->dsub)) return fail(IVFADC_ERR_STATE, "no matrix-core table kernels for m=%d dsub=%d", h->m, h->dsub);
    TRY(set_device(h));
    const int m = h->m;
    DevBuf dq, dt, df;
    int rc = dq.ensure((size_t)h->d * 4);
    if (rc == IVFADC_OK) rc = dt.ensure((size_t)m * 256);
    if (rc == IVFADC_OK) rc = df.ensure((size_t)(3 + 2 * m) * 4);
    if (rc == IVFADC_OK) {
        hipError_t e = hipMemcpyAsync(dq.p, query, (size_t)h->d * 4, hipMemcpyHostToDevice, h->stream);
        if (e == hipSuccess) {
            const size_t lds = lb_lds_bytes(m, h->dsub, 1);
            void (*dk)(const IndexView, const LbView, const float *, int, unsigned char *, float *) =
                (m == 48) ? lb_debug_kernel<48, 16> : lb_debug_kernel<16, 6>;
            rc = fn_raise_lds(h->device, (const void *)dk, lds, false);
            if (rc == IVFADC_OK) {
                hipLaunchKernelGGL(dk, dim3(1), dim3(256), lds, h->stream, index_view(h), lb_view(h), dq.as<float>(), cell, dt.as<unsigned char>(),
                                   df.as<float>());
                e = hipGetLastError();
            }
        }
        if (e == hipSuccess) e = hipMemcpyAsync(out_table, dt.p, (size_t)m * 256, hipMemcpyDeviceToHost, h->stream);
        if (e == hipSuccess) e = hipMemcpyAsync(out_consts, df.p, (size_t)(3 + 2 * m) * 4, hipMemcpyDeviceToHost, h->stream);
        if (e == hipSuccess) e = hipStreamSynchronize(h->stream);
        if (e != hipSuccess && rc == IVFADC_OK) rc = fail(IVFADC_ERR_HIP, "debug table: %s", hipGetErrorString(e));
    }
    dq.release(); dt.release(); df.release();
    return rc;
} IVF_CATCH

int ivfadc_set_workspace_limit(ivfadc_t *h, uint64_t bytes)
try {
    HandleLock lk_(h);
    if (!h) return fail(IVFADC_ERR_INVALID, "null handle");
    h->ws_budget = (size_t)std::max<uint64_t>(bytes, 1 << 20);
    return IVFADC_OK;
} IVF_CATCH

int ivfadc_set_tuning(ivfadc_t *h, int qg, int chunk_points)
try {
    HandleLock lk_(h);
    if (!h) return fail(IVFADC_ERR_INVALID, "null handle");
    if (!(qg == 0 || qg == -1 || qg == -2 || qg == -3 || qg == 1 || qg == 2 || qg == 4 || qg == 8))
        return fail(IVFADC_ERR_INVALID, "qg must be 0, -1, -2, -3, 1, 2, 4 or 8");
// ... 243 lines not shown
```

ivfadc.jl_amd/csrc/kernels.hip.h:

```cpp
#pragma once
#include <hip/hip_runtime.h>
#include <stdint.h>
#include <type_traits>
#include "wave_sort.hip.h"

typedef unsigned long long u64;
typedef unsigned int u32;
typedef float v2f __attribute__((ext_vector_type(2)));
typedef float v4f __attribute__((ext_vector_type(4)));

#define KEY_MAX 0xFFFFFFFFFFFFFFFFull


namespace ivf {

static __device__ __forceinline__ int lane_id()
{
    return (int)__builtin_amdgcn_mbcnt_hi(~0u, __builtin_amdgcn_mbcnt_lo(~0u, 0u));
}

static __device__ __forceinline__ void wave_sync()
{
    __builtin_amdgcn_fence(__ATOMIC_RELEASE, "wavefront");
    __builtin_amdgcn_wave_barrier();
// ... 1336 lines not shown
        __syncthreads();
    }
    u64 *buf = sbuf + (size_t)wv * cap;
    const int Ksel = APPROX ? approx_pool(w) : w;
    WSel<SMALL> sel;
    sel.init(KEY_MAX, buf, cap, Ksel);
    const float *row = cdist + (size_t)q * kc;
    bool tiled = false, listed = false;
    int cnt = 0;
    if constexpr (APPROX && SMALL && WPQ == 1) {
        if (rf.tlist) {
            listed = true;
            const WSel<true> ex = select_listed(q, w, rf, lane, (int *)buf);
            cnt = ex.finish(w, lane);
            wave_sync();
            ex.store(buf, cnt, lane);
        } else if (rf.tmin)
            tiled = select_row_tiled(sel, row, rf.tmin + (size_t)q * rf.ntiles, rf.ntiles, rf.tile_w, kc, Ksel, lane, (int *)buf);
    }
    if (!listed) {
    bool shortrow = false;
    if constexpr (WPQ == 4 && SMALL) {
        if (Ksel <= SHORT_ROW_MAXK && kc <= 2048 && (kc & 3) == 0) {
            __shared__ u64 s_wb[4];
            __shared__ u32 s_cc;
            shortrow = select_row_short<APPROX>(sel, row, kc, Ksel, wv, lane, (int)threadIdx.x, sbuf, s_wb, &s_cc);
            if (shortrow && wv != 0) return;
        }
    }
    if (!tiled && !shortrow) select_row<APPROX, WPQ>(sel, row, kc, Ksel, wv, lane, WPQ == 4 ? &s_thr : (u64 *)nullptr);
    cnt = sel.finish(Ksel, lane);
    if (shortrow) wave_sync();
    sel.store(buf, cnt, lane);
    if (WPQ == 4 && !shortrow) {
        if (lane == 0) s_cnt[wv] = cnt;
        __syncthreads();
        if (wv != 0) return;
        merge_waves(sel, sbuf, (size_t)cap, s_cnt, 1, Ksel, KEY_MAX, 0, lane);
        cnt = sel.finish(Ksel, lane);
        sel.store(buf, cnt, lane);
    }
    if constexpr (APPROX && SMALL) {
        const WSel<true> ex = refine_probes(sel, cnt, w, q, rf, lane);
        cnt = ex.finish(w, lane);
        wave_sync();
        ex.store(buf, cnt, lane);
    }
    }
    wave_sync();
    u32 running = 0, mine_total = 0;
    for (int j0 = 0; j0 < cnt; j0 += 64) {
        const int j = j0 + lane;
        u32 len = 0;
        int l = 0;
        float dd = 0.0f;
        if (j < cnt) {
            const u64 key = buf[j];
            l = (int)(u32)key;
            dd = __uint_as_float((u32)(key >> 32));
            len = list_len[l];
        }
        const bool mine = nparts <= 1 || (l % nparts) == part;
        u32 incl = len, minc = mine ? len : 0u;
#pragma unroll
        for (int off = 1; off < 64; off <<= 1) {
            const u32 v = __shfl_up(incl, off);
            if (lane >= off) incl += v;
        }
#pragma unroll
        for (int off = 32; off > 0; off >>= 1) minc += __shfl_xor(minc, off);
        if (j < cnt) {
            const size_t o = (size_t)q * w + j;
            probe_list[o] = l;
            probe_dc[o] = dd;
            probe_base[o] = running + incl - len;
            if (list_cnt && mine) atomicAdd(&list_cnt[l], 1u);
        }
        running += __shfl(incl, 63);
        mine_total += minc;
    }
    if (lane == 0) atomicAdd(scanned_points + (size_t)(q & 63) * 8, (u64)mine_total);
}

__global__ __launch_bounds__(256) void probe_ingest_kernel(const int *__restrict__ src_list, const float *__restrict__ src_dc, int nq, int kc,
                                                           int w, const u32 *__restrict__ list_len, int *__restrict__ probe_list,
                                                           float *__restrict__ probe_dc, u32 *__restrict__ probe_base,
                                                           u32 *__restrict__ list_cnt, u32 *__restrict__ totals,
                                                           u64 *__restrict__ scanned_points)
{
    const int lane = threadIdx.x & 63, wv = threadIdx.x >> 6;
    const int q = blockIdx.x * 4 + wv;
    if (q >= nq) return;
    u32 running = 0;
    for (int j0 = 0; j0 < w; j0 += 64) {
        const int j = j0 + lane;
        const size_t o = (size_t)q * w + j;
        u32 len = 0;
        int l = 0;
        float dd = 0.0f;
        if (j < w) {
            l = min(max(src_list[o], 0), kc - 1);
            dd = src_dc[o];
            if (__float_as_uint(dd) > 0x7F7FFFFFu) dd = 0.0f;
            len = list_len[l];
        }
        u32 incl = len;
#pragma unroll
        for (int off = 1; off < 64; off <<= 1) {
            const u32 v = __shfl_up(incl, off);
            if (lane >= off) incl += v;
        }
        if (j < w) {
            probe_list[o] = l;
            probe_dc[o] = dd;
            probe_base[o] = running + incl - len;
            if (list_cnt) atomicAdd(&list_cnt[l], 1u);
        }
        running += __shfl(incl, 63);
    }
    if (lane == 0) {
        if (totals) totals[q] = running;
        atomicAdd(scanned_points + (size_t)(q & 63) * 8, (u64)running);
    }
}

__global__ __launch_bounds__(1024) void bucket_scan_kernel(const u32 *__restrict__ list_cnt, const u32 *__restrict__ list_len,
                                                           int kc, int QG, u32 CH, u32 *__restrict__ bucket_off,
                                                           u32 *__restrict__ wi_off, u32 *__restrict__ cursor,
                                                           u32 *__restrict__ queue_head, u32 *__restrict__ item_list = nullptr)
{
    __shared__ u32 sa[1024], sb[1024];
    const int tid = threadIdx.x;
    const int per = (kc + 1023) / 1024;
    const int l0 = tid * per, l1 = min(kc, l0 + per);
    u32 suma = 0, sumb = 0;
    for (int l = l0; l < l1; ++l) {
        const u32 cnt = list_cnt[l];
        const u32 len = list_len[l];
        const u32 ng = (cnt + QG - 1) / QG;
        const u32 nch = (len + CH - 1) / CH;
        suma += cnt;
        sumb += ng * nch;
    }
    sa[tid] = suma;
    sb[tid] = sumb;
    __syncthreads();
    for (int off = 1; off < 1024; off <<= 1) {
        u32 va = 0, vb = 0;
        if (tid >= off) { va = sa[tid - off]; vb = sb[tid - off]; }
        __syncthreads();
        sa[tid] += va;
        sb[tid] += vb;
        __syncthreads();
    }
    u32 runa = sa[tid] - suma, runb = sb[tid] - sumb;
    for (int l = l0; l < l1; ++l) {
        const u32 cnt = list_cnt[l];
        const u32 len = list_len[l];
        const u32 ng = (cnt + QG - 1) / QG;
        const u32 nch = (len + CH - 1) / CH;
        bucket_off[l] = runa;
        wi_off[l] = runb;
        cursor[l] = 0;
        if (item_list)
            for (u32 i = 0; i < ng * nch; ++i) item_list[runb + i] = (u32)l;
        runa += cnt;
        runb += ng * nch;
    }
    if (tid == 1023) { bucket_off[kc] = sa[1023]; wi_off[kc] = sb[1023]; queue_head[0] = 0; }
}

__global__ __launch_bounds__(256) void bucket_scatter_kernel(const int *__restrict__ probe_list, int nprobe,
                                                             const u32 *__restrict__ bucket_off, u32 *__restrict__ cursor,
                                                             u32 *__restrict__ bucket_items, int nparts, int part)
{
    const int p = blockIdx.x * 256 + threadIdx.x;
    if (p >= nprobe) return;
    const int l = probe_list[p];
    if (nparts > 1 && (l % nparts) != part) return;
    const u32 pos = bucket_off[l] + atomicAdd(&cursor[l], 1u);
    bucket_items[pos] = (u32)p;
}

struct IndexView {
    const float *centroids;
// ... 1152 lines not shown
                if (pred) key = part_keys[slot * K + i];
            }
            pred = pred && key < sel.thr();
            sel.push(pred, key, K, lane);
        }
    } else
    for (int j = 0; j < w; ++j) {
        const size_t pi = (size_t)q * w + j;
        const int l = probe_list[pi];
        if (nparts > 1 && (l % nparts) != part) continue;
        const u32 len = list_len[l];
        const int nch = (int)((len + CH - 1) / CH);
        const int tot = nch * K;
        for (int e0 = 0; e0 < tot; e0 += 64) {
            const int e = e0 + lane;
            bool pred = e < tot;
            u64 key = KEY_MAX;
            if (pred) {
                const int c = e / K, i = e - c * K;
                const size_t slot = pi * maxch + c;
                pred = (u32)i < part_cnt[slot];
                if (pred) key = part_keys[slot * K + i];
            }
            pred = pred && key < sel.thr();
            sel.push(pred, key, K, lane);
        }
    }
    const int cnt = sel.finish(K, lane);
    if (out_keys) sel.for_each(cnt, lane, [&](int i, u64 key) { out_keys[(size_t)q * K + i] = key; });
    else sel.for_each(cnt, lane, [&](int i, u64 key) {
        emit_result(key, i, q, w, K, probe_list + (size_t)q * w, probe_base + (size_t)q * w, list_pos, ids, out_ids, out_dists);
    });
    if (lane == 0) {
        out_counts[q] = cnt;
        qthr[q] = KEY_MAX;
    }
}

template <bool SMALL>
__global__ __launch_bounds__(256) void partial_merge_kernel(int nq, int w, int K, int cap, int nranks, const u64 *__restrict__ keys,
                                                            size_t rank_stride_u64, const int *__restrict__ counts, size_t rank_stride_i32,
                                                            const int *__restrict__ probe_list, const u32 *__restrict__ probe_base,
                                                            const int64_t *__restrict__ list_pos, const u32 *__restrict__ ids,
                                                            u32 *__restrict__ out_ids, float *__restrict__ out_dists, int *__restrict__ out_counts)
{
    extern __shared__ __attribute__((aligned(16))) unsigned char smem_raw[];
    u64 *sbuf = (u64 *)smem_raw;
    const int lane = threadIdx.x & 63, wv = threadIdx.x >> 6;
    const int q = blockIdx.x * 4 + wv;
    if (q >= nq) return;
    WSel<SMALL> sel;
    sel.init(KEY_MAX, sbuf + (size_t)wv * cap, cap, K);
    for (int r = 0; r < nranks; ++r) {
        const int c = counts[(size_t)r * rank_stride_i32 + q];
        sel_absorb(sel, keys + (size_t)r * rank_stride_u64 + (size_t)q * K, c < K ? c : K, K, lane);
    }
    const int cnt = sel.finish(K, lane);
    sel.for_each(cnt, lane, [&](int i, u64 key) {
        emit_result(key, i, q, w, K, probe_list + (size_t)q * w, probe_base + (size_t)q * w, list_pos, ids, out_ids, out_dists);
    });
    if (lane == 0) out_counts[q] = cnt;
}

#include "lbscan.hip.h"
#include "nfscan.hip.h"
#include "wg8scan.hip.h"

struct QScanArgs {
    IndexView ix;
    LbView lb;
    const float *queries;
    int nq, w, K, cap;
    const int *probe_list;
    const float *probe_dc;
    const u32 *probe_base;
    u32 *out_ids;
    float *out_dists;
    int *out_counts;
    int prune;
    const float *cdist;
    u64 *scanned_points;
    int approx;
    RefineArgs rf;
};

template <int M, int DS, int PG, bool SMALL, bool LB = false>
static __device__ __forceinline__ void qscan_body(const QScanArgs &a, unsigned char *smem_raw, const int q)
{
    const IndexView &ix = a.ix;
    const int tid = threadIdx.x, lane = tid & 63, wv = tid >> 6;
    const int m = (M > 0) ? M : ix.m;
    const int K = a.K, cap = a.cap, w = a.w;
    static_assert(!LB || (SMALL && M > 0 && DS > 0), "LB rounds: compile-time shape, register selectors");
    LdsCarve L = carve_lds<PG, SMALL, 1>(smem_raw, m, ix.d, cap);
    int stage_floats = (m < 2 ? 2 : m) * 256 * PG;
    if constexpr (LB) {
        using C = LbCfg<M, DS, PG>;
        stage_floats = (int)(C::TAB_BYTES / 4u);
        L.tab = (float *)smem_raw;
        L.resid = nullptr;
        L.selbuf = nullptr;
        L.xch = (u64 *)smem_raw;
        L.xcap = 64;
        L.scnt = (int *)(smem_raw + C::END);
        L.swi = (u32 *)(L.scnt + 4 * PG);
        L.sthr = (u64 *)(L.swi + 4);
    }

    WSel<SMALL> sel[1];
    sel[0].init(KEY_MAX, SMALL ? nullptr : L.selbuf + (size_t)wv * cap, cap, K);
    if (tid == 0) arm_bound<1>(L.sthr, 0, KEY_MAX);

    const int *prow_list = a.probe_list + (size_t)q * w;
    const float *prow_dc = a.probe_dc + (size_t)q * w;
    const u32 *prow_base = a.probe_base + (size_t)q * w;
    const bool cached = w <= 32;
    const int PW = cached ? 32 : 64;
    int *s_list = (int *)(L.sthr + STHR_WORDS * PG);
    float *s_dc = (float *)(s_list + PW);
    u32 *s_base = (u32 *)(s_dc + PW);
    u32 *s_len = s_base + PW;
    u32 *s_coff = s_len + PW;
    if (a.cdist) {
        const int Ksel = a.approx ? approx_pool(w) : w;
        WSel<true> ws;
        ws.init(KEY_MAX, nullptr, 64, Ksel);
        const float *row = a.cdist + (size_t)q * ix.kc;
        __syncthreads();
        bool have = false;
        if constexpr (LB && M > 16) {
            if (Ksel <= SHORT_ROW_MAXK && ix.kc > 2048 && ix.kc <= 8192 && (ix.kc & 3) == 0) {
                u64 *wbound = (u64 *)(s_list + 160);
                u32 *ccnt = (u32 *)(s_list + 168);
                if (ix.kc <= 4096)
                    have = a.approx ? select_row_short<true, 4>(ws, row, ix.kc, Ksel, wv, lane, tid, L.xch, wbound, ccnt)
                                    : select_row_short<false, 4>(ws, row, ix.kc, Ksel, wv, lane, tid, L.xch, wbound, ccnt);
                else
                    have = a.approx ? select_row_short<true, 8>(ws, row, ix.kc, Ksel, wv, lane, tid, L.xch, wbound, ccnt)
                                    : select_row_short<false, 8>(ws, row, ix.kc, Ksel, wv, lane, tid, L.xch, wbound, ccnt);
            }
        }
        if (!have && Ksel <= SHORT_ROW_MAXK && ix.kc <= 2048 && (ix.kc & 3) == 0) {
            u64 *wbound = (u64 *)(s_list + 160);
            u32 *ccnt = (u32 *)(s_list + 168);
            have = a.approx ? select_row_short<true>(ws, row, ix.kc, Ksel, wv, lane, tid, L.xch, wbound, ccnt)
                            : select_row_short<false>(ws, row, ix.kc, Ksel, wv, lane, tid, L.xch, wbound, ccnt);
        }
        if constexpr (M > 16) {
        if (!have && a.approx && a.rf.tmin != nullptr) {
            int *flag = s_list + 170;
            if (wv == 0) {
                const bool ok = select_row_tiled(ws, row, a.rf.tmin + (size_t)q * a.rf.ntiles, a.rf.ntiles, a.rf.tile_w, ix.kc, Ksel, lane,
                                                 (int *)L.xch);
                if (lane == 0) *flag = ok ? 1 : 0;
            }
            __syncthreads();
            have = *flag != 0;
        }
        }
        if (!have) {
            if (a.approx) select_row<true, 4>(ws, row, ix.kc, Ksel, wv, lane, L.sthr);
            else select_row<false, 4>(ws, row, ix.kc, Ksel, wv, lane, L.sthr);
            const int wc = ws.finish(Ksel, lane);
            ws.store(L.xch + (size_t)wv * 64, wc, lane);
            if (lane == 0) L.scnt[wv] = wc;
            __syncthreads();
        }
        int fc = 0;
        if (wv == 0) {
            if (lane == 0) arm_bound<1>(L.sthr, 0, KEY_MAX);
            if (!have) merge_waves(ws, L.xch, (size_t)64, L.scnt, 1, Ksel, KEY_MAX, 0, lane);
            fc = ws.finish(Ksel, lane);
        }
        if (a.approx) {
            ws = refine_probes_wg<(M > 16)>(ws, fc, w, q, a.rf, wv, lane, tid, L.tab, stage_floats, s_list);
            if (wv == 0) fc = ws.finish(w, lane);
        }
        if (wv == 0) {
            u32 len = 0;
            int l = 0;
            if (lane < fc) {
                l = (int)(u32)ws.top;
                len = ix.list_len[l];
            }
            u32 incl = len;
#pragma unroll
            for (int off = 1; off < 64; off <<= 1) {
                const u32 v = __shfl_up(incl, off);
                if (lane >= off) incl += v;
            }
            if (lane < fc) {
                s_list[lane] = l;
                s_dc[lane] = __uint_as_float((u32)(ws.top >> 32));
                s_base[lane] = incl - len;
                if (cached) {
                    s_len[lane] = len;
                    s_coff[lane] = (u32)(ix.list_codeoff[l] >> 8);
                }
            }
            const u32 total = __shfl(incl, 63);
            if (lane == 0) atomicAdd(a.scanned_points + (size_t)(q & 63) * 8, (u64)total);
        }
        __syncthreads();
        prow_list = s_list;
        prow_dc = s_dc;
        prow_base = s_base;
    } else if (cached) {
        if (tid < w) {
            const int l = prow_list[tid];
            s_list[tid] = l;
            s_dc[tid] = prow_dc[tid];
            s_base[tid] = prow_base[tid];
            s_len[tid] = ix.list_len[l];
            s_coff[tid] = (u32)(ix.list_codeoff[l] >> 8);
        }
        __syncthreads();
        prow_list = s_list;
        prow_dc = s_dc;
        prow_base = s_base;
    }
    if constexpr (LB) {
        lb_rounds<M, DS, PG>(ix, a.lb, a.queries, smem_raw, q, w, K, a.prune, a.scanned_points, sel[0], L.sthr, s_list, s_dc, s_base, s_len, s_coff, wv,
                             lane, tid);
    } else {
    constexpr int RU = (M > 0 && M * DS * PG <= 256) ? 1 : 2;
    constexpr bool can_pipe = M == 0 || M * DS * PG <= 256 * RU;
    const bool pipe = can_pipe && cached && ix.d * PG <= 256 * RU;
    float rq[RU], rc[RU];
    auto resid_fetch = [&](int j0) {
#pragma unroll
        for (int u = 0; u < RU; ++u) {
            const int e = tid + u * 256;
            rq[u] = 0.0f;
            rc[u] = 0.0f;
            if (e < ix.d * PG) {
                const int i = e / PG, sl = e - i * PG;
                const int pj = (j0 + sl) < w ? j0 + sl : j0;
                rq[u] = a.queries[(size_t)q * ix.d + i];
                rc[u] = ix.centroids[(size_t)prow_list[pj] * ix.d + i];
            }
        }
    };
    auto resid_store = [&]() {
#pragma unroll
        for (int u = 0; u < RU; ++u) {
            const int e = tid + u * 256;
            if (e < ix.d * PG) L.resid[e] = rq[u] - rc[u];
        }
    };
    if (pipe) {
        resid_fetch(0);
        resid_store();
    }
    int np = PG;
    for (int j0 = 0; j0 < w; j0 += np) {
        np = PG;
        int li[PG], qi[PG];
        u32 len[PG], sb[PG];
        float dcv[PG];
        const uint8_t *cb[PG];
#pragma unroll
        for (int s = 0; s < PG; ++s) {
            const bool ok = (j0 + s) < w;
            const int pj = ok ? j0 + s : j0;
            li[s] = prow_list[pj];
            qi[s] = q;
            dcv[s] = prow_dc[pj];
            sb[s] = prow_base[pj];
            if (cached) {
                len[s] = ok ? s_len[pj] : 0u;
                cb[s] = ix.codes + ((size_t)s_coff[pj] << 8);
            } else {
                len[s] = ok ? ix.list_len[li[s]] : 0u;
                cb[s] = ix.codes + ix.list_codeoff[li[s]];
            }
        }
        CodeRegs<M, ppl_of<M, 1>()> cr[PG];
#pragma unroll
        for (int s = 0; s < PG; ++s) scan_prefetch(cr[s], cb[s], 0u, len[s], wv, lane);
        __syncthreads();
        if (a.prune) {
            const u32 thi = (u32)(readfirstlane64(L.sthr[0]) >> 32);
            if (__float_as_uint(dcv[0]) > thi) {
                if (a.prune == 1) {
                    if (tid == 0) {
                        u64 skipped = 0;
                        for (int pj = j0; pj < w; ++pj) skipped += cached ? s_len[pj] : ix.list_len[prow_list[pj]];
                        atomicAdd(a.scanned_points + (size_t)(q & 63) * 8 + 1, skipped);
                    }
// ... 14 lines not shown
                for (int s = 0; s < PG; ++s) none = none && len[s] == 0;
                if (none) {
                    if (pipe && (j0 + np) < w) {
                        resid_fetch(j0 + np);
                        resid_store();
                    }
                    continue;
                }
            }
            if constexpr (PG == 2 && SMALL) {
                if (j0 == 0 && w > 1 && len[1] != 0 && dcv[1] > 2.0f * dcv[0]) {
                    len[1] = 0;
                    np = 1;
                }
            }
        }
        const int ns = (PG == 2 && len[1 % PG] == 0) ? 1 : PG;
        constexpr bool PKB = M == 48 && DS == 16 && PG == 1;
        const bool pkb = PKB && ix.codebooks_p != nullptr;
        if (!pipe) {
            if (pkb) {
                for (int i = tid; i < ix.d; i += 256) {
                    const int ii = i / DS, t = i - ii * DS;
                    L.resid[((ii >> 1) * DS + t) * 2 + (ii & 1)] = a.queries[(size_t)q * ix.d + i] - ix.centroids[(size_t)li[0] * ix.d + i];
                }
            } else {
                build_residuals<PG>(ix, a.queries, qi, li, L.resid, tid);
            }
            __syncthreads();
        }
        if constexpr (M == 48 && DS == 16) {
            if (pkb) build_tables_pk<DS>(ix, m, L.resid, L.tab, tid);
            else build_tables_deep<PG, DS, 4>(ix, m, L.resid, L.tab, tid);
        } else {
            if constexpr (PG == 2 && DS > 0) {
                if (ns == 1) build_tables_t<PG, DS, TAB_SEP, 0, true>(ix, m, L.resid, L.tab, tid);
                else build_tables_t<PG, DS, TAB_SEP>(ix, m, L.resid, L.tab, tid);
            } else build_tables_t<PG, DS, TAB_SEP>(ix, m, L.resid, L.tab, tid);
        }
        __syncthreads();
        const bool more = pipe && (j0 + np) < w;
        if (more) resid_fetch(j0 + np);
        __builtin_amdgcn_s_setprio(3);
        if constexpr (PG == 2 && M > 0 && M <= 16 && SMALL) {
            scan_pair<M>(0u, (u32)M * 1024u, cb[0], cb[1], len[0], len[1], dcv[0], dcv[1], sb[0], sb[1], sel, K, wv, lane, cr[0], cr[1],
                         L.sthr);
        } else {
#pragma unroll
            for (int s = 0; s < PG; ++s) {
                if (len[s] == 0) continue;
                const float dc1[1] = {dcv[s]};
                const u32 sb1[1] = {sb[s]};
                scan_range<M, 1>(L.tab + (size_t)s * m * 256, (u32)s * (u32)m * 1024u, cb[s], ix.cs, m, 0u, len[s], dc1, sb1, 1, sel, K, wv,
                                 lane, cr[s], L.sthr);
            }
        }
        __builtin_amdgcn_s_setprio(0);
        if (more) resid_store();
    }
    }
    const int mycnt = sel[0].finish(K, lane);
    __syncthreads();
    sel[0].store(L.xch + (size_t)wv * L.xcap, mycnt, lane);
    if (lane == 0) L.scnt[wv] = mycnt;
    __syncthreads();
    if (wv == 0) {
        merge_waves(sel[0], L.xch, (size_t)L.xcap, L.scnt, 1, K, KEY_MAX, 0, lane);
        const int fc = sel[0].finish(K, lane);
        sel[0].for_each(fc, lane, [&](int i, u64 key) {
            emit_result(key, i, q, w, K, prow_list, prow_base, ix.list_pos, ix.ids, a.out_ids, a.out_dists);
        });
        if (lane == 0) a.out_counts[q] = fc;
    }
}

template <int M, int DS, int PG, bool SMALL, bool LB = false>
__global__ __launch_bounds__(256, LB ? (M <= 16 ? 3 : (PG >= 4 ? 2 : (PG == 3 ? 3 : 4))) : 1) void qscan_kernel(const QScanArgs a)
{
    extern __shared__ __attribute__((aligned(16))) unsigned char smem_raw[];
    qscan_body<M, DS, PG, SMALL, LB>(a, smem_raw, (int)blockIdx.x);
}

constexpr int RIDER_QW = 4;
struct CoarseNext {
    const float *queries;
    float *out;
    int nq, ncx;
};
template <int M, int DS, int PG>
__global__ __launch_bounds__(256) void qscan_coarse_kernel(const QScanArgs a, const CoarseNext cn)
{
    extern __shared__ __attribute__((aligned(16))) unsigned char smem_raw[];
    if ((int)blockIdx.x < a.nq) {
        qscan_body<M, DS, PG, true, false>(a, smem_raw, (int)blockIdx.x);
    } else {
        const int t = (int)blockIdx.x - a.nq;
        coarse_sgpr_tile<RIDER_QW>(cn.queries, a.ix.centroids, cn.out, cn.nq, a.ix.kc, a.ix.d, t % cn.ncx, t / cn.ncx, (float *)smem_raw);
    }
}

#include "smallq.hip.h"

__global__ __launch_bounds__(256) void encode_kernel(const float *__restrict__ pts, const int *__restrict__ assign, int d, int m,
                                                     int ksub, int dsub, const float *__restrict__ centroids,
                                                     const float *__restrict__ codebooks, const uint8_t *__restrict__ labels,
                                                     uint8_t *__restrict__ out_codes)
{
    extern __shared__ __attribute__((aligned(16))) unsigned char smem_raw[];
    float *resid = (float *)smem_raw;
    u64 *best = (u64 *)(resid + (((size_t)d + 3) & ~(size_t)3));
    const int p = blockIdx.x, tid = threadIdx.x;
    const int l = assign[p];
    for (int i = tid; i < d; i += 256) resid[i] = pts[(size_t)p * d + i] - centroids[(size_t)l * d + i];
    for (int i = tid; i < m; i += 256) best[i] = KEY_MAX;
    __syncthreads();
    for (int e = tid; e < m * 256; e += 256) {
        const int ii = e >> 8, c = e & 255;
        u64 key = KEY_MAX;
        if (c < ksub) {
            const float *cw = codebooks + ((size_t)ii * ksub + c) * dsub;
            const float *rr = resid + (size_t)ii * dsub;
            float sum = 0.0f;
            for (int t = 0; t < dsub; ++t) {
                const float df = cw[t] - rr[t];
                sum = sum + df * df;
            }
            key = make_key(sum, (u32)c);
        }
#pragma unroll
        for (int off = 32; off > 0; off >>= 1) {
            const u64 o = __shfl_xor(key, off);
            key = o < key ? o : key;
        }
        if ((tid & 63) == 0) atomicMin(&best[ii], key);
    }
    __syncthreads();
    for (int i = tid; i < m; i += 256) out_codes[(size_t)p * m + i] = labels[i * ksub + (int)(u32)best[i]];
}

__global__ __launch_bounds__(256) void argmin_rows_kernel(const float *__restrict__ cdist, int n, int kc, int *__restrict__ out)
{
    const int lane = threadIdx.x & 63, wv = threadIdx.x >> 6;
    const int r = blockIdx.x * 4 + wv;
    if (r >= n) return;
    const float *row = cdist + (size_t)r * kc;
    u64 key = KEY_MAX;
    for (int c = lane; c < kc; c += 64) {
        const u64 k2 = make_key(row[c], (u32)c);
        key = k2 < key ? k2 : key;
    }
#pragma unroll
    for (int off = 32; off > 0; off >>= 1) {
        const u64 o = __shfl_xor(key, off);
        key = o < key ? o : key;
    }
    if (lane == 0) out[r] = (int)(u32)key;
}

static __device__ __forceinline__ u64 mix64(u64 x)
{
    x ^= x >> 30; x *= 0xBF58476D1CE4E5B9ull;
    x ^= x >> 27; x *= 0x94D049BB133111EBull;
    x ^= x >> 31;
    return x;
}

__global__ __launch_bounds__(256) void synth_codes_kernel(uint8_t *__restrict__ codes, const int64_t *__restrict__ list_pos,
                                                          const u32 *__restrict__ list_len,
                                                          const int64_t *__restrict__ list_codeoff, int kc, int m, int cs,
                                                          u64 seed)
{
    const int l = blockIdx.x;
    const int64_t lpos = list_pos[l];
    const int64_t len = list_len[l];
    const int64_t ndw = len * (cs >> 2);
    u32 *dst = (u32 *)(codes + list_codeoff[l]);
    const int dpp = cs >> 2;
// ... 107 lines not shown
```

ivfadc.jl_amd/index.py:

```python
import ctypes as C
import math
import threading

import numpy as np

from . import _native as nat
from . import trainer

DEFAULT_COARSE_K = 2
DEFAULT_QUANTIZATION_K = 256
DEFAULT_QUANTIZATION_M = 1
DEFAULT_QUANTIZATION_METHOD = "pq"
DEFAULT_COARSE_DISTANCE = "SqEuclidean"
DEFAULT_COARSE_QUANTIZER = "naive"
DEFAULT_QUANTIZATION_DISTANCE = "SqEuclidean"
DEFAULT_COARSE_MAXITER = 25
DEFAULT_QUANTIZATION_MAXITER = 25

_TYPE_TO_BITS = {np.dtype(np.uint8): 8, np.dtype(np.uint16): 16, np.dtype(np.uint32): 32}
_JULIA_NAMES = {np.dtype(np.uint8): "UInt8", np.dtype(np.uint16): "UInt16", np.dtype(np.uint32): "UInt32"}


class NaiveQuantizer:

# ... 264 lines not shown
    def _io(self, nq, ka):
        pin = getattr(self, "_pin", None)
        if pin is None or pin[0].a.size < nq * self.d or pin[1].a.size < nq * ka or pin[3].a.size < nq:
            grow = lambda old, need: max(need + need // 2, old)
            o = [0, 0, 0] if pin is None else [pin[0].a.size, pin[1].a.size, pin[3].a.size]
            self._pin = None
            pin = (nat.PinnedArray(grow(o[0], nq * self.d), np.float32), nat.PinnedArray(grow(o[1], nq * ka), np.uint32),
                   nat.PinnedArray(grow(o[1], nq * ka), np.float32), nat.PinnedArray(grow(o[2], nq), np.int32))
            self._pin = pin
        return (pin[0].a[:nq * self.d].reshape(nq, self.d), pin[1].a[:nq * ka].reshape(nq, ka), pin[2].a[:nq * ka].reshape(nq, ka),
                pin[3].a[:nq])

    def search_raw(self, queries, k, w=1):
        q = np.ascontiguousarray(queries, np.float32)
        assert q.ndim == 2 and q.shape[1] == self.d, "queries must be (nq, %d)" % self.d
        nq = q.shape[0]
        ka = max(int(k), 1)
        ids = np.zeros((nq, ka), np.uint32)
        dists = np.full((nq, ka), np.inf, np.float32)
        counts = np.zeros(nq, np.int32)
        nat.check(nat.lib().ivfadc_search(self._h, nq, nat.ptr(q, C.c_float), int(k), int(w), nat.ptr(ids, C.c_uint32),
                                          nat.ptr(dists, C.c_float), nat.ptr(counts, C.c_int32)))
        return ids, dists, counts

    def coarse_search_raw(self, queries, w):
        q = np.ascontiguousarray(queries, np.float32)
        assert q.ndim == 2 and q.shape[1] == self.d, "queries must be (nq, %d)" % self.d
        nq, wa = q.shape[0], max(int(w), 1)
        lists = np.zeros((nq, wa), np.int32)
        dists = np.zeros((nq, wa), np.float32)
        nat.check(nat.lib().ivfadc_coarse_search(self._h, nq, nat.ptr(q, C.c_float), int(w), nat.ptr(lists, C.c_int32),
                                                 nat.ptr(dists, C.c_float)))
        return lists, dists

    def search_preassigned_raw(self, queries, k, lists, dists):
        q = np.ascontiguousarray(queries, np.float32)
        assert q.ndim == 2 and q.shape[1] == self.d, "queries must be (nq, %d)" % self.d
        nq = q.shape[0]
        pl = np.ascontiguousarray(lists, np.int32)
        pd = np.ascontiguousarray(dists, np.float32)
        assert pl.ndim == 2 and pl.shape[0] == nq and pd.shape == pl.shape, "lists and dists must both be (nq, w)"
        ka = max(int(k), 1)
        ids = np.zeros((nq, ka), np.uint32)
        out = np.full((nq, ka), np.inf, np.float32)
        counts = np.zeros(nq, np.int32)
        nat.check(nat.lib().ivfadc_search_preassigned(self._h, nq, nat.ptr(q, C.c_float), int(k), int(pl.shape[1]), nat.ptr(pl, C.c_int32),
                                                      nat.ptr(pd, C.c_float), nat.ptr(ids, C.c_uint32), nat.ptr(out, C.c_float),
                                                      nat.ptr(counts, C.c_int32)))
        return ids, out, counts

    def coarse_search_device(self, nq, q_ptr, w, lists_ptr, dists_ptr):
        nat.check(nat.lib().ivfadc_coarse_search_device(self._h, int(nq), C.c_void_p(q_ptr), int(w), C.c_void_p(lists_ptr),
                                                        C.c_void_p(dists_ptr)))

    def search_device_preassigned(self, nq, q_ptr, k, w, lists_ptr, cdists_ptr, ids_ptr, dists_ptr, counts_ptr):
        nat.check(nat.lib().ivfadc_search_device_preassigned(self._h, int(nq), C.c_void_p(q_ptr), int(k), int(w), C.c_void_p(lists_ptr),
                                                             C.c_void_p(cdists_ptr), C.c_void_p(ids_ptr), C.c_void_p(dists_ptr),
                                                             C.c_void_p(counts_ptr)))

    def set_profiling(self, on):
        nat.check(nat.lib().ivfadc_set_profiling(self._h, int(on)))

    def reset_stats(self):
        nat.check(nat.lib().ivfadc_reset_stats(self._h))

    def get_stats(self):
        st = nat.Stats()
        nat.check(nat.lib().ivfadc_get_stats(self._h, C.byref(st)))
        return {f: getattr(st, f) for f, _ in nat.Stats._fields_}

    def set_tuning(self, qg=0, chunk_points=0):
        nat.check(nat.lib().ivfadc_set_tuning(self._h, int(qg), int(chunk_points)))

    def set_coarse_mode(self, mode):
        nat.check(nat.lib().ivfadc_set_coarse_mode(self._h, int(mode)))

    def set_pruning(self, on):
        nat.check(nat.lib().ivfadc_set_pruning(self._h, int(bool(on))))

    def set_next_queries(self, nq, d_queries_ptr, token):
        nat.check(nat.lib().ivfadc_set_next_queries(self._h, int(nq), C.c_void_p(d_queries_ptr) if d_queries_ptr else None,
                                                    C.c_uint64(int(token))))

    def set_query_token(self, token):
        nat.check(nat.lib().ivfadc_set_query_token(self._h, C.c_uint64(int(token))))

    def search_batches_raw(self, batches, k, w=1):
        qs = [np.asarray(b, np.float32).reshape(-1, self.d) for b in batches]
        sizes = np.array([q.shape[0] for q in qs], np.int64)
        total = int(sizes.sum())
        ka = max(int(k), 1)
        with self._io_lock():
            allq, ids, dists, counts = self._io(total, ka)
            s = 0
            for q in qs:
                allq[s:s + q.shape[0]] = q
                s += q.shape[0]
            nat.check(nat.lib().ivfadc_search_batches(self._h, len(qs), nat.ptr(sizes, C.c_int64), nat.ptr(allq, C.c_float), int(k), int(w),
                                                      nat.ptr(ids, C.c_uint32), nat.ptr(dists, C.c_float), nat.ptr(counts, C.c_int32)))
            out, s = [], 0
            for n in sizes.tolist():
                out.append((ids[s:s + n].copy(), dists[s:s + n].copy(), counts[s:s + n].copy()))
                s += n
        return out

    def set_table_mode(self, mode):
        nat.check(nat.lib().ivfadc_set_table_mode(self._h, int(mode)))

    def set_u16_tables(self, mode):
        nat.check(nat.lib().ivfadc_set_u16_tables(self._h, int(mode)))

    def debug_lb_table(self, query, cell):
        q = np.ascontiguousarray(query, np.float32)
        tab = np.zeros((self.m, 256), np.uint8)
        cf = np.zeros(3 + 2 * self.m, np.float32)
        nat.check(nat.lib().ivfadc_debug_lb_table(self._h, q.ctypes.data_as(C.POINTER(C.c_float)), int(cell),
                                                  tab.ctypes.data_as(C.POINTER(C.c_uint8)), cf.ctypes.data_as(C.POINTER(C.c_float))))
        return tab, float(cf[0]), float(cf[1]), float(cf[2]), cf[3:3 + self.m].copy(), cf[3 + self.m:].copy()

    def set_workspace_limit(self, nbytes):
        nat.check(nat.lib().ivfadc_set_workspace_limit(self._h, C.c_uint64(int(nbytes))))

    def sync(self):
        nat.check(nat.lib().ivfadc_sync(self._h))

    def set_stream(self, hip_stream):
        nat.check(nat.lib().ivfadc_set_stream(self._h, C.c_void_p(int(hip_stream))))

    def search_device(self, nq, q_ptr, k, w, ids_ptr, dists_ptr, counts_ptr):
        nat.check(nat.lib().ivfadc_search_device(self._h, int(nq), C.c_void_p(q_ptr), int(k), int(w), C.c_void_p(ids_ptr),
                                                 C.c_void_p(dists_ptr), C.c_void_p(counts_ptr)))


def _comm_methods():
    def comm_init(self, nranks, rank, id128):
        buf = np.ascontiguousarray(id128, np.uint8)
        assert buf.shape == (128,)
        nat.check(nat.lib().ivfadc_comm_init(self._h, int(nranks), int(rank), nat.ptr(buf, C.c_uint8)))

    def search_device_allgather_on(self, searcher, nq, q_ptr, k, w, block_ptr, gathered_ptr, slot):
        nat.check(nat.lib().ivfadc_search_device_allgather_on(self._h, searcher._h, int(nq), C.c_void_p(q_ptr), int(k), int(w),
                                                             C.c_void_p(block_ptr), C.c_void_p(gathered_ptr), int(slot)))

    def search_device_allgather(self, nq, q_ptr, k, w, block_ptr, gathered_ptr, slot):
        nat.check(nat.lib().ivfadc_search_device_allgather(self._h, int(nq), C.c_void_p(q_ptr), int(k), int(w), C.c_void_p(block_ptr),
                                                          C.c_void_p(gathered_ptr), int(slot)))

    def comm_wait(self):
        n = C.c_int64(0)
        nat.check(nat.lib().ivfadc_comm_wait(self._h, C.byref(n)))
        return int(n.value)

    def set_list_partition(self, nparts, part):
        nat.check(nat.lib().ivfadc_set_list_partition(self._h, int(nparts), int(part)))

    def search_device_partial(self, nq, q_ptr, k, w, keys_ptr, counts_ptr):
        nat.check(nat.lib().ivfadc_search_device_partial(self._h, int(nq), C.c_void_p(q_ptr), int(k), int(w), C.c_void_p(keys_ptr), C.c_void_p(counts_ptr)))

    def merge_partials_device(self, nq, k, nparts, keys_all_ptr, counts_all_ptr, ids_ptr, dists_ptr, counts_ptr):
        nat.check(nat.lib().ivfadc_merge_partials_device(self._h, int(nq), int(k), int(nparts), C.c_void_p(keys_all_ptr), C.c_void_p(counts_all_ptr),
                                                         C.c_void_p(ids_ptr), C.c_void_p(dists_ptr), C.c_void_p(counts_ptr)))

    def search_device_listpart(self, nq, q_ptr, k, w, block_ptr, gathered_ptr, ids_ptr, dists_ptr, counts_ptr):
        nat.check(nat.lib().ivfadc_search_device_listpart(self._h, int(nq), C.c_void_p(q_ptr), int(k), int(w), C.c_void_p(block_ptr),
                                                          C.c_void_p(gathered_ptr), C.c_void_p(ids_ptr), C.c_void_p(dists_ptr), C.c_void_p(counts_ptr)))

# ... 153 lines not shown
```

Measured before the change: 49.78 million.

## Add probe-list rider that computes next batch's top-w coarse probes in scan kernel

```diff
diff --git a/include/ivfadc_hip.h b/include/ivfadc_hip.h
--- a/include/ivfadc_hip.h
+++ b/include/ivfadc_hip.h
@@ -180,6 +180,7 @@
 int ivfadc_set_pruning(ivfadc_t *h, int on);
 
 int ivfadc_set_next_queries(ivfadc_t *h, int64_t nq, const float *d_queries, uint64_t token);
+int ivfadc_get_rider_info(ivfadc_t *h, int *rider_form, int *probe_source);
 int ivfadc_set_query_token(ivfadc_t *h, uint64_t token);
 
 int ivfadc_set_table_mode(ivfadc_t *h, int mode);
diff --git a/ivfadc.jl_amd/_native.py b/ivfadc.jl_amd/_native.py
--- a/ivfadc.jl_amd/_native.py
+++ b/ivfadc.jl_amd/_native.py
@@ -111,6 +111,7 @@
     L.ivfadc_set_pruning.argtypes = [vp, C.c_int]
     L.ivfadc_set_next_queries.argtypes = [vp, C.c_int64, C.c_void_p, C.c_uint64]
     L.ivfadc_set_query_token.argtypes = [vp, C.c_uint64]
+    L.ivfadc_get_rider_info.argtypes = [vp, C.POINTER(C.c_int), C.POINTER(C.c_int)]
     L.ivfadc_search_batches.argtypes = [vp, C.c_int, i64p, fp, C.c_int, C.c_int, u32p, fp, i32p]
     L.ivfadc_set_table_mode.argtypes = [vp, C.c_int]
     L.ivfadc_set_u16_tables.argtypes = [vp, C.c_int]
@@ -164,7 +165,7 @@
                  "mg_num_devices", "mg_set_gather", "mg_collectives", "set_list_partition", "search_device_partial", "merge_partials_device", "search_device_listpart", "comm_unique_id", "comm_init", "search_device_allgather", "search_device_allgather_on", "clone_view", "comm_wait", "comm_destroy"):
         getattr(L, "ivfadc_" + name).restype = C.c_int
     for name in ("create", "set_lists", "synth_lists", "encode", "append", "search", "search_device", "sync", "set_stream",
-                 "ntotal", "get_lists", "set_profiling", "reset_stats", "get_stats", "set_tuning", "set_workspace_limit", "set_coarse_mode", "set_pruning", "set_table_mode", "set_next_queries", "set_query_token", "search_batches", "save_index", "load_index", "delete_ids", "shift_ids"):
+                 "ntotal", "get_lists", "set_profiling", "reset_stats", "get_stats", "set_tuning", "set_workspace_limit", "set_coarse_mode", "set_pruning", "set_table_mode", "set_next_queries", "set_query_token", "get_rider_info", "search_batches", "save_index", "load_index", "delete_ids", "shift_ids"):
         getattr(L, "ivfadc_" + name).restype = C.c_int
     _lib = L
     return L
diff --git a/ivfadc.jl_amd/csrc/ivfadc_hip.hip b/ivfadc.jl_amd/csrc/ivfadc_hip.hip
--- a/ivfadc.jl_amd/csrc/ivfadc_hip.hip
+++ b/ivfadc.jl_amd/csrc/ivfadc_hip.hip
@@ -354,6 +354,11 @@
     uint64_t hint_token = 0, pf_token = 0, cur_token = 0, own_token = 0;
     hipEvent_t hint_ev = nullptr;
     DevBuf cdist2;
+    DevBuf pp_list, pp_dc, pp_list2, pp_dc2;
+    int pf_form = 0, avail_form = 0, pp_P = 0;
+    bool probe_riders = false;
+    int pp_use = 0;
+    int last_rider_form = 0, last_probe_source = 0;
     DevBuf pre_list, pre_dc;
     DevBuf q_stage, cdist, probe_list, probe_dc, probe_base, list_cnt, bucket_off, wi_off, cursor, bucket_items, misc,
         qthr, part_keys, part_cnt, out_ids, out_dists, out_counts, assign, enc_codes, pts_stage, dbg;
@@ -1164,17 +1169,32 @@
     const bool pre = pre_list != nullptr;
     u64 *d_scanned = h->misc.as<u64>();
     const bool wpq4 = !pl.lanes && nb * 1 < (int64_t)8 * h->num_cu * 4 && h->kc >= 512 && !(pl.form == ScanForm::QueryMajorLb && !pl.fuse_topw);
-    const bool have_rows = single && !pre && !pl.coarse_mfma && !pl.twolevel && h->avail_q == d_q && h->avail_nq == nb && h->cdist2.p != nullptr;
+    const bool standing = single && !pre && !pl.coarse_mfma && !pl.twolevel && h->avail_q == d_q && h->avail_nq == nb;
+    const bool have_rows = standing && h->avail_form == 0 && h->cdist2.p != nullptr;
+    const bool have_probes = standing && h->avail_form == 1 && w <= h->pp_P && h->pp_list2.p != nullptr && h->pp_dc2.p != nullptr && !h->u16 &&
+                             h->part_n <= 1;
     h->avail_q = nullptr;
-    if (pre || pl.twolevel || have_rows) {
+    h->pp_use = 0;
+    if (pre || pl.twolevel || have_rows || have_probes) {
         h->tmin_tiles = 0;
         h->last_listed = false;
     }
     if (pre) {
-        hipLaunchKernelGGL(probe_ingest_kernel, dim3((unsigned)((nb + 3) / 4)), dim3(256), 0, h->stream, pre_list, pre_dc, (int)nb, h->kc, w,
+        hipLaunchKernelGGL(probe_ingest_kernel, dim3((unsigned)((nb + 3) / 4)), dim3(256), 0, h->stream, pre_list, pre_dc, w, (int)nb, h->kc, w,
                            h->list_len.as<u32>(), h->probe_list.as<int>(), h->probe_dc.as<float>(), h->probe_base.as<u32>(), lc, (u32 *)nullptr,
                            d_scanned);
         HIP_TRY(hipGetLastError());
+    } else if (have_probes) {
+        std::swap(h->pp_list, h->pp_list2);
+        std::swap(h->pp_dc, h->pp_dc2);
+        const bool direct = pl.form == ScanForm::QueryMajor && pl.small_k && w <= 32;
+        h->pp_use = direct ? 1 : 2;
+        if (!direct) {
+            hipLaunchKernelGGL(probe_ingest_kernel, dim3((unsigned)((nb + 3) / 4)), dim3(256), 0, h->stream, h->pp_list.as<int>(),
+                               h->pp_dc.as<float>(), h->pp_P, (int)nb, h->kc, w, h->list_len.as<u32>(), h->probe_list.as<int>(),
+                               h->probe_dc.as<float>(), h->probe_base.as<u32>(), lc, (u32 *)nullptr, d_scanned);
+            HIP_TRY(hipGetLastError());
+        }
     } else if (pl.twolevel) {
         TRY(run_twolevel(h, d_q, nb, w, h->probe_list.as<int>(), h->probe_dc.as<float>(), h->probe_base.as<u32>(), lc, d_scanned));
     } else if (have_rows) {
@@ -1183,11 +1203,12 @@
         TRY(run_coarse(h, d_q, nb, pl.coarse_mfma, pl.coarse_mfma && (pl.fuse_topw ? h->m > 16 : !wpq4),
                        !pl.fuse_topw && !wpq4, w));
     }
-    if (!pl.fuse_topw && !pl.twolevel && !pre)
+    if (!pl.fuse_topw && !pl.twolevel && !pre && !have_probes)
         TRY(launch_topw(h, d_q, nb, w, pl.capw, pl.coarse_mfma, wpq4, h->probe_list.as<int>(), h->probe_dc.as<float>(), h->probe_base.as<u32>(), lc,
                         d_scanned, h->part_n, h->part_i));
     h->stats.last_rider = 0;
-    h->stats.coarse_prefetched = have_rows ? 1 : 0;
+    h->stats.coarse_prefetched = (have_rows || have_probes) ? 1 : 0;
+    h->last_probe_source = have_rows ? 1 : (have_probes ? 1 + h->pp_use : 0);
     h->stats.last_twolevel = pl.twolevel ? 1 : 0;
     h->stats.coarse_mfma = pl.coarse_mfma ? 1 : 0;
     h->stats.coarse_f16 = (pl.coarse_mfma && h->last_coarse_f16 && !have_rows) ? 1 : 0;
@@ -1206,7 +1227,11 @@
     a.nq = (int)nb; a.w = w; a.K = K; a.cap = pl.cap;
     a.probe_list = h->probe_list.as<int>(); a.probe_dc = h->probe_dc.as<float>(); a.probe_base = h->probe_base.as<u32>();
     a.out_ids = d_ids; a.out_dists = d_dists; a.out_counts = d_counts;
-    a.cdist = pl.fuse_topw ? h->cdist.as<float>() : (const float *)nullptr;
+    a.cdist = (pl.fuse_topw && h->pp_use == 0) ? h->cdist.as<float>() : (const float *)nullptr;
+    a.pp_list = h->pp_use == 1 ? h->pp_list.as<int>() : (const int *)nullptr;
+    a.pp_dc = h->pp_use == 1 ? h->pp_dc.as<float>() : (const float *)nullptr;
+    a.pp_stride = h->pp_P;
+    h->pp_use = 0;
     a.scanned_points = h->misc.as<u64>();
     a.approx = pl.coarse_mfma ? 1 : 0;
     a.rf = refine_args(h, d_q);
@@ -1219,13 +1244,27 @@
                       (!h->allow_mfma || kc < h->mfma_min_kc) && (h->hint_nq + 4 * RIDER_QW - 1) / (4 * RIDER_QW) <= 65535 &&
                       (size_t)h->hint_nq * kc * 4 <= h->ws_budget / 4;
     qscan_coarse_fn_t fk = ride ? pick_qscan_coarse(h->m, h->dsub, pl.qg) : nullptr;
+    const bool probe_riders = ride && h->probe_riders && (h->d & 3) == 0 && kc >= 128;
     if (fk) {
-        TRY(h->cdist2.ensure((size_t)h->hint_nq * kc * 4));
         CoarseNext cn;
-        cn.queries = h->hint_q; cn.out = h->cdist2.as<float>(); cn.nq = (int)h->hint_nq; cn.ncx = (kc + 63) / 64;
+        cn.queries = h->hint_q; cn.nq = (int)h->hint_nq; cn.ncx = (kc + 63) / 64;
+        cn.out = nullptr; cn.probes = probe_riders ? 1 : 0; cn.P = std::min(kc, RIDER_P);
+        cn.cnorm = h->cnorm.as<float>(); cn.out_list = nullptr; cn.out_dc = nullptr;
+        cn.rf = refine_args(h, h->hint_q);
+        cn.rf.eps_coef = 2.0f * (float)(h->d + 3) * 5.9604645e-8f;
+        cn.rf.qflags = nullptr; cn.rf.tlist = nullptr; cn.rf.tmin = nullptr;
+        if (probe_riders) {
+            TRY(h->pp_list2.ensure((size_t)h->hint_nq * cn.P * 4));
+            TRY(h->pp_dc2.ensure((size_t)h->hint_nq * cn.P * 4));
+            cn.out_list = h->pp_list2.as<int>(); cn.out_dc = h->pp_dc2.as<float>();
+        } else {
+            TRY(h->cdist2.ensure((size_t)h->hint_nq * kc * 4));
+            cn.out = h->cdist2.as<float>();
+        }
         const size_t lds = std::max<size_t>(pl.lds, (size_t)64 * 132 * 4);
         TRY(fn_raise_lds(h->device, (const void *)fk, lds, true));
-        const unsigned grid = (unsigned)(nb + (int64_t)cn.ncx * ((h->hint_nq + 4 * RIDER_QW - 1) / (4 * RIDER_QW)));
+        const unsigned grid = probe_riders ? (unsigned)(nb + (h->hint_nq + 3) / 4)
+                                           : (unsigned)(nb + (int64_t)cn.ncx * ((h->hint_nq + 4 * RIDER_QW - 1) / (4 * RIDER_QW)));
         if (h->hint_ev) {
             HIP_TRY(hipStreamWaitEvent(h->stream, h->hint_ev, 0));
             h->hint_ev = nullptr;
@@ -1237,7 +1276,10 @@
         h->pf_q = h->hint_q;
         h->pf_nq = h->hint_nq;
         h->pf_token = h->hint_token;
+        h->pf_form = probe_riders ? 1 : 0;
+        if (probe_riders) h->pp_P = cn.P;
         h->stats.last_rider = 1;
+        h->last_rider_form = probe_riders ? 2 : 1;
     } else {
         if (h->profiling) TRY(ev_begin(h, 0, ep));
         hipLaunchKernelGGL((qscan_fn_t)pl.fn, dim3((unsigned)nb), dim3(pl.threads), pl.lds, h->stream, a);
@@ -1498,7 +1540,7 @@
         TRY(h->gen_tot.ensure((size_t)na * 4));
         if (pre_list) {
             hipLaunchKernelGGL(probe_ingest_kernel, dim3((unsigned)((na + 3) / 4)), dim3(256), 0, h->stream, pre_list + (size_t)a0 * w,
-                               pre_dc + (size_t)a0 * w, (int)na, kc, w, h->list_len.as<u32>(), h->probe_list.as<int>(), h->probe_dc.as<float>(),
+                               pre_dc + (size_t)a0 * w, w, (int)na, kc, w, h->list_len.as<u32>(), h->probe_list.as<int>(), h->probe_dc.as<float>(),
                                h->probe_base.as<u32>(), (u32 *)nullptr, h->gen_tot.as<u32>(), d_scanned);
             HIP_TRY(hipGetLastError());
         } else {
@@ -1789,9 +1831,13 @@
     const bool declared = h->cur_token != 0 && h->cur_token == h->pf_token;
     h->avail_q = declared ? h->pf_q : nullptr;
     h->avail_nq = declared ? h->pf_nq : 0;
-    h->pf_q = nullptr; h->pf_nq = 0; h->pf_token = 0; h->cur_token = 0;
+    h->avail_form = h->pf_form;
+    h->pf_q = nullptr; h->pf_nq = 0; h->pf_token = 0; h->cur_token = 0; h->pf_form = 0;
     h->stats.coarse_prefetched = 0;
     h->stats.last_rider = 0;
+    h->last_rider_form = 0;
+    h->last_probe_source = 0;
+    h->pp_use = 0;
     h->partial_nq = -1;
     TRY(set_device(h));
     if (h->dirty) TRY(upload_lists(h));
@@ -1825,9 +1871,11 @@
 int coarse_dev(ivfadc_index *h, int64_t nq, const float *d_q, int w, int32_t *d_lists, float *d_dists)
 {
     HintScope hint_scope{h};
-    h->pf_q = nullptr; h->pf_nq = 0; h->pf_token = 0; h->cur_token = 0;
+    h->pf_q = nullptr; h->pf_nq = 0; h->pf_token = 0; h->cur_token = 0; h->pf_form = 0;
     h->stats.coarse_prefetched = 0;
     h->stats.last_rider = 0;
+    h->last_rider_form = 0;
+    h->last_probe_source = 0;
     h->partial_nq = -1;
     TRY(set_device(h));
     if (h->dirty) TRY(upload_lists(h));
@@ -2421,7 +2469,7 @@
     if (h->comm || h->comm_stream) (void)ivfadc_comm_destroy(h);
     for (auto &ep : h->pending) { (void)hipEventDestroy(ep.a); (void)hipEventDestroy(ep.b); }
     for (auto &ep : h->free_ev) { (void)hipEventDestroy(ep.a); (void)hipEventDestroy(ep.b); }
-    DevBuf *bufs[] = {&h->lb_f16, &h->lb_isc, &h->cent_f16, &h->q_f16, &h->q_flags, &h->tl_centres, &h->tl_off, &h->tl_rad, &h->tl_cent, &h->tl_slot, &h->tl_gdist, &h->cdist2, &h->pre_list, &h->pre_dc, &h->cent_t, &h->sq_keys, &h->sq_cnt, &h->sq_arrive, &h->lb_split, &h->lb_n2, &h->lb_lab, &h->lb_maxn, &h->nf_n2, &h->nf_lab, &h->wg8_tabs, &h->wg8_items, &h->centroids, &h->codebooks, &h->codebooks_t, &h->codebooks_p, &h->labels, &h->cnorm, &h->tmin, &h->tlist, &h->cent_hi, &h->cent_lo, &h->q_hi, &h->q_lo, &h->gen_a, &h->gen_b, &h->gen_tmp, &h->gen_off, &h->gen_tot, &h->list_pos, &h->list_len, &h->list_codeoff, &h->codes, &h->ids, &h->app_stage, &h->q_stage,
+    DevBuf *bufs[] = {&h->lb_f16, &h->lb_isc, &h->cent_f16, &h->q_f16, &h->q_flags, &h->tl_centres, &h->tl_off, &h->tl_rad, &h->tl_cent, &h->tl_slot, &h->tl_gdist, &h->cdist2, &h->pp_list, &h->pp_dc, &h->pp_list2, &h->pp_dc2, &h->pre_list, &h->pre_dc, &h->cent_t, &h->sq_keys, &h->sq_cnt, &h->sq_arrive, &h->lb_split, &h->lb_n2, &h->lb_lab, &h->lb_maxn, &h->nf_n2, &h->nf_lab, &h->wg8_tabs, &h->wg8_items, &h->centroids, &h->codebooks, &h->codebooks_t, &h->codebooks_p, &h->labels, &h->cnorm, &h->tmin, &h->tlist, &h->cent_hi, &h->cent_lo, &h->q_hi, &h->q_lo, &h->gen_a, &h->gen_b, &h->gen_tmp, &h->gen_off, &h->gen_tot, &h->list_pos, &h->list_len, &h->list_codeoff, &h->codes, &h->ids, &h->app_stage, &h->q_stage,
                       &h->cdist, &h->probe_list, &h->probe_dc, &h->probe_base, &h->list_cnt, &h->bucket_off, &h->wi_off, &h->cursor,
                       &h->bucket_items, &h->misc, &h->qthr, &h->part_keys, &h->part_cnt, &h->out_ids, &h->out_dists, &h->out_counts,
                       &h->assign, &h->enc_codes, &h->pts_stage, &h->dbg};
@@ -2494,7 +2542,7 @@
                         &v->lb_maxn, &v->nf_n2, &v->nf_lab, &v->cent_t, &v->cent_hi, &v->cent_lo, &v->list_pos, &v->list_len, &v->list_codeoff,
                         &v->codes, &v->ids};
     for (DevBuf *b : shared) b->alias();
-    DevBuf *scratch[] = {&v->wg8_tabs, &v->wg8_items, &v->q_f16, &v->q_flags, &v->tl_gdist, &v->cdist2, &v->pre_list, &v->pre_dc, &v->sq_keys, &v->sq_cnt, &v->sq_arrive, &v->tmin, &v->tlist, &v->q_hi, &v->q_lo, &v->gen_a, &v->gen_b, &v->gen_tmp,
+    DevBuf *scratch[] = {&v->wg8_tabs, &v->wg8_items, &v->q_f16, &v->q_flags, &v->tl_gdist, &v->cdist2, &v->pp_list, &v->pp_dc, &v->pp_list2, &v->pp_dc2, &v->pre_list, &v->pre_dc, &v->sq_keys, &v->sq_cnt, &v->sq_arrive, &v->tmin, &v->tlist, &v->q_hi, &v->q_lo, &v->gen_a, &v->gen_b, &v->gen_tmp,
                          &v->gen_off, &v->gen_tot, &v->app_stage, &v->q_stage, &v->cdist, &v->probe_list, &v->probe_dc, &v->probe_base, &v->list_cnt,
                          &v->bucket_off, &v->wi_off, &v->cursor, &v->bucket_items, &v->misc, &v->qthr, &v->part_keys, &v->part_cnt, &v->out_ids,
                          &v->out_dists, &v->out_counts, &v->assign, &v->enc_codes, &v->pts_stage, &v->dbg};
@@ -2532,6 +2580,8 @@
     v->hint_q = v->pf_q = v->avail_q = nullptr;
     v->hint_nq = v->pf_nq = v->avail_nq = 0;
     v->hint_token = v->pf_token = v->cur_token = 0;
+    v->pf_form = v->avail_form = v->pp_P = v->pp_use = 0;
+    v->last_rider_form = v->last_probe_source = 0;
     v->partial_keys = nullptr;
     v->partial_nq = -1;
     v->qthr_armed = 0;
@@ -2571,7 +2621,7 @@
     dst->wg8_mode = src->wg8_mode; dst->wg8_wide = src->wg8_wide; dst->u16_wide = src->u16_wide; dst->u16_tables = src->u16_tables;
     dst->allow_nf = src->allow_nf; dst->allow_sq = src->allow_sq; dst->sq_inside = src->sq_inside; dst->allow_lb = src->allow_lb;
     dst->force_lb = src->force_lb; dst->allow_bf16 = src->allow_bf16; dst->allow_f16 = src->allow_f16; dst->lb_use_f16 = src->lb_use_f16; dst->allow_prune = src->allow_prune; dst->allow_listed = src->allow_listed;
-    dst->allow_filt = src->allow_filt; dst->allow_mfma = src->allow_mfma; dst->mfma_min_kc = src->mfma_min_kc; dst->ws_budget = src->ws_budget;
+    dst->allow_filt = src->allow_filt; dst->probe_riders = src->probe_riders; dst->allow_mfma = src->allow_mfma; dst->mfma_min_kc = src->mfma_min_kc; dst->ws_budget = src->ws_budget;
     dst->force_qg = src->force_qg; dst->force_chunk = src->force_chunk;
     dst->part_n = src->part_n; dst->part_i = src->part_i;
     dst->tl_use = src->tl_use && dst->tl_cent.p != nullptr; dst->tl_mode = src->tl_mode;
@@ -4216,7 +4266,8 @@
 try {
     HandleLock lk_(h);
     if (!h) return fail(IVFADC_ERR_INVALID, "null handle");
-    if (mode < 0 || mode > 8) return fail(IVFADC_ERR_INVALID, "mode must be 0 ... 8");
+    if (mode < 0 || mode > 9) return fail(IVFADC_ERR_INVALID, "mode must be 0 ... 9");
+    h->probe_riders = mode == 9;
     h->allow_f16 = mode != 8 && mode != 3;
     h->tl_mode = mode == 6 ? 1 : (mode == 7 ? -1 : 0);
     if (h->tl_tried) h->tl_use = h->tl_G > 0 && (h->tl_mode > 0 || (h->tl_mode == 0 && h->tl_probe_fraction >= 0.f && h->tl_probe_fraction <= 0.02f));
@@ -4245,6 +4296,15 @@
     h->hint_q = (nq > 0 && token != 0) ? d_queries : nullptr;
     h->hint_nq = h->hint_q ? nq : 0;
     h->hint_token = h->hint_q ? token : 0;
+    return IVFADC_OK;
+} IVF_CATCH
+
+int ivfadc_get_rider_info(ivfadc_t *h, int *rider_form, int *probe_source)
+try {
+    HandleLock lk_(h);
+    if (!h) return fail(IVFADC_ERR_INVALID, "null handle");
+    if (rider_form) *rider_form = h->last_rider_form;
+    if (probe_source) *probe_source = h->last_probe_source;
     return IVFADC_OK;
 } IVF_CATCH
 
diff --git a/ivfadc.jl_amd/csrc/kernels.hip.h b/ivfadc.jl_amd/csrc/kernels.hip.h
--- a/ivfadc.jl_amd/csrc/kernels.hip.h
+++ b/ivfadc.jl_amd/csrc/kernels.hip.h
@@ -1442,8 +1442,8 @@
     if (lane == 0) atomicAdd(scanned_points + (size_t)(q & 63) * 8, (u64)mine_total);
 }
 
-__global__ __launch_bounds__(256) void probe_ingest_kernel(const int *__restrict__ src_list, const float *__restrict__ src_dc, int nq, int kc,
-                                                           int w, const u32 *__restrict__ list_len, int *__restrict__ probe_list,
+__global__ __launch_bounds__(256) void probe_ingest_kernel(const int *__restrict__ src_list, const float *__restrict__ src_dc, int src_stride,
+                                                           int nq, int kc, int w, const u32 *__restrict__ list_len, int *__restrict__ probe_list,
                                                            float *__restrict__ probe_dc, u32 *__restrict__ probe_base,
                                                            u32 *__restrict__ list_cnt, u32 *__restrict__ totals,
                                                            u64 *__restrict__ scanned_points)
@@ -1454,13 +1454,13 @@
     u32 running = 0;
     for (int j0 = 0; j0 < w; j0 += 64) {
         const int j = j0 + lane;
-        const size_t o = (size_t)q * w + j;
+        const size_t o = (size_t)q * w + j, so = (size_t)q * src_stride + j;
         u32 len = 0;
         int l = 0;
         float dd = 0.0f;
         if (j < w) {
-            l = min(max(src_list[o], 0), kc - 1);
-            dd = src_dc[o];
+            l = min(max(src_list[so], 0), kc - 1);
+            dd = src_dc[so];
             if (__float_as_uint(dd) > 0x7F7FFFFFu) dd = 0.0f;
             len = list_len[l];
         }
@@ -2779,6 +2779,9 @@
     u64 *scanned_points;
     int approx;
     RefineArgs rf;
+    const int *pp_list;
+    const float *pp_dc;
+    int pp_stride;
 };
 
 template <int M, int DS, int PG, bool SMALL, bool LB = false>
@@ -2902,6 +2905,36 @@
         prow_list = s_list;
         prow_dc = s_dc;
         prow_base = s_base;
+    } else if (a.pp_list) {
+        if (wv == 0) {
+            u32 len = 0;
+            int l = 0;
+            float dcl = 0.0f;
+            if (lane < w) {
+                l = min(max(a.pp_list[(size_t)q * a.pp_stride + lane], 0), ix.kc - 1);
+                dcl = a.pp_dc[(size_t)q * a.pp_stride + lane];
+                len = ix.list_len[l];
+            }
+            u32 incl = len;
+#pragma unroll
+            for (int off = 1; off < 32; off <<= 1) {
+                const u32 v = __shfl_up(incl, off);
+                if (lane >= off) incl += v;
+            }
+            if (lane < w) {
+                s_list[lane] = l;
+                s_dc[lane] = dcl;
+                s_base[lane] = incl - len;
+                s_len[lane] = len;
+                s_coff[lane] = (u32)(ix.list_codeoff[l] >> 8);
+            }
+            const u32 total = __shfl(incl, 31);
+            if (lane == 0) atomicAdd(a.scanned_points + (size_t)(q & 63) * 8, (u64)total);
+        }
+        __syncthreads();
+        prow_list = s_list;
+        prow_dc = s_dc;
+        prow_base = s_base;
     } else if (cached) {
         if (tid < w) {
             const int l = prow_list[tid];
@@ -3082,17 +3115,161 @@
 }
 
 constexpr int RIDER_QW = 4;
+constexpr int RIDER_P = SHORT_ROW_MAXK;
 struct CoarseNext {
     const float *queries;
     float *out;
     int nq, ncx;
+    int probes, P;
+    const float *cnorm;
+    int *out_list;
+    float *out_dc;
+    RefineArgs rf;
 };
+
+static __device__ __forceinline__ void coarse_probe_tile(const CoarseNext &cn, const float *__restrict__ Cn, int kc, int d, int tile,
+                                                         unsigned char *smem_raw)
+{
+    constexpr int PLD = 16, PDK = 16;
+    static_assert((4 * 64 * PLD + 4 * 1024) * 4 <= 64 * CSQ_LD * 4, "the probe rider's carve exceeds the LDS a rider launch requests");
+    const int tid = threadIdx.x, lane = tid & 63;
+    const int wv = __builtin_amdgcn_readfirstlane(tid >> 6);
+    float *ws = (float *)smem_raw + (size_t)wv * 64 * PLD;
+    float *S = (float *)smem_raw + 4 * 64 * PLD;
+    const int nq = cn.nq, P = cn.P;
+    const int Ksel = approx_pool(P);
+    const int myq = tile * 4 + wv;
+    const int qj = min(tile * 4 + (lane & 3), nq - 1);
+    const float *qrow = cn.queries + (size_t)qj * d;
+    const int srow = lane >> 2, sp = lane & 3;
+    const int wsw = (sp ^ ((srow >> 2) & 3)) * 4;
+    const int rsw = (lane >> 2) & 3;
+    WSel<true> sel;
+    sel.init(KEY_MAX, nullptr, 64, Ksel);
+    for (int cb = 0; cb < kc; cb += 1024) {
+        const int c0 = cb + wv * 256;
+        const int ns = __builtin_amdgcn_readfirstlane(min(4, max(0, (kc - c0 + 63) >> 6)));
+        struct CIn { v4f c0, c1, c2, c3; };
+        struct QIn { v4f q0, q1, q2, q3; };
+        const int nk = (d + PDK - 1) / PDK;
+        const int T = ns * nk;
+        auto fetch_c = [&](int t) -> CIn {
+            const int s = t / nk, k0 = (t - s * nk) * PDK;
+            const int rem = d - k0;
+            const int off = 4 * sp < rem ? 4 * sp : 0;
+            const int r0 = c0 + s * 64 + srow;
+            CIn n;
+            n.c0 = *(const v4f *)(Cn + (size_t)min(r0, kc - 1) * d + k0 + off);
+            n.c1 = *(const v4f *)(Cn + (size_t)min(r0 + 16, kc - 1) * d + k0 + off);
+            n.c2 = *(const v4f *)(Cn + (size_t)min(r0 + 32, kc - 1) * d + k0 + off);
+            n.c3 = *(const v4f *)(Cn + (size_t)min(r0 + 48, kc - 1) * d + k0 + off);
+            return n;
+        };
+        auto fetch_q = [&](int t) -> QIn {
+            const int s = t / nk, k0 = (t - s * nk) * PDK;
+            const int rem = d - k0;
+            QIn n;
+            n.q0 = *(const v4f *)(qrow + k0);
+            n.q1 = *(const v4f *)(qrow + k0 + (4 < rem ? 4 : 0));
+            n.q2 = *(const v4f *)(qrow + k0 + (8 < rem ? 8 : 0));
+            n.q3 = *(const v4f *)(qrow + k0 + (12 < rem ? 12 : 0));
+            return n;
+        };
+        if (cb) __syncthreads();
+        v4f acc = (v4f){0.f, 0.f, 0.f, 0.f};
+        QIn qn = fetch_q(0);
+        auto step = [&](CIn &cin, int t_) {
+            const bool live = t_ < T;
+            const int t = live ? t_ : T - 1;
+            const int s = t / nk, k0 = (t - s * nk) * PDK;
+            const int rem = live ? d - k0 : 0;
+            wave_sync();
+            *(v4f *)&ws[srow * PLD + wsw] = cin.c0;
+            *(v4f *)&ws[(srow + 16) * PLD + wsw] = cin.c1;
+            *(v4f *)&ws[(srow + 32) * PLD + wsw] = cin.c2;
+            *(v4f *)&ws[(srow + 48) * PLD + wsw] = cin.c3;
+            const v4f z = (v4f){0.f, 0.f, 0.f, 0.f};
+            const v4f b0 = 0 < rem ? qn.q0 : z, b1 = 4 < rem ? qn.q1 : z, b2 = 8 < rem ? qn.q2 : z, b3 = 12 < rem ? qn.q3 : z;
+            wave_sync();
+            qn = fetch_q(min(t_ + 1, T - 1));
+            cin = fetch_c(min(t_ + 2, T - 1));
+            const float *ar = &ws[lane * PLD];
+            const v4f a0 = *(const v4f *)(ar + ((0 ^ rsw) << 2)), a1 = *(const v4f *)(ar + ((1 ^ rsw) << 2)),
+                      a2 = *(const v4f *)(ar + ((2 ^ rsw) << 2)), a3 = *(const v4f *)(ar + ((3 ^ rsw) << 2));
+            v4f x = acc;
+            x = __builtin_amdgcn_mfma_f32_4x4x1f32(a0.x, b0.x, x, 0, 0, 0);
+            x = __builtin_amdgcn_mfma_f32_4x4x1f32(a0.y, b0.y, x, 0, 0, 0);
+            x = __builtin_amdgcn_mfma_f32_4x4x1f32(a0.z, b0.z, x, 0, 0, 0);
+            x = __builtin_amdgcn_mfma_f32_4x4x1f32(a0.w, b0.w, x, 0, 0, 0);
+            x = __builtin_amdgcn_mfma_f32_4x4x1f32(a1.x, b1.x, x, 0, 0, 0);
+            x = __builtin_amdgcn_mfma_f32_4x4x1f32(a1.y, b1.y, x, 0, 0, 0);
+            x = __builtin_amdgcn_mfma_f32_4x4x1f32(a1.z, b1.z, x, 0, 0, 0);
+            x = __builtin_amdgcn_mfma_f32_4x4x1f32(a1.w, b1.w, x, 0, 0, 0);
+            x = __builtin_amdgcn_mfma_f32_4x4x1f32(a2.x, b2.x, x, 0, 0, 0);
+            x = __builtin_amdgcn_mfma_f32_4x4x1f32(a2.y, b2.y, x, 0, 0, 0);
+            x = __builtin_amdgcn_mfma_f32_4x4x1f32(a2.z, b2.z, x, 0, 0, 0);
+            x = __builtin_amdgcn_mfma_f32_4x4x1f32(a2.w, b2.w, x, 0, 0, 0);
+            x = __builtin_amdgcn_mfma_f32_4x4x1f32(a3.x, b3.x, x, 0, 0, 0);
+            x = __builtin_amdgcn_mfma_f32_4x4x1f32(a3.y, b3.y, x, 0, 0, 0);
+            x = __builtin_amdgcn_mfma_f32_4x4x1f32(a3.z, b3.z, x, 0, 0, 0);
+            x = __builtin_amdgcn_mfma_f32_4x4x1f32(a3.w, b3.w, x, 0, 0, 0);
+            acc = x;
+            if (live && k0 + PDK >= d) {
+                const int cl = wv * 256 + s * 64 + (lane >> 2) * 4;
+                float v[4];
+#pragma unroll
+                for (int r = 0; r < 4; ++r) {
+                    const int c = cb + cl + r;
+                    v[r] = c < kc ? cn.cnorm[c] - 2.0f * x[r] : __builtin_inff();
+                }
+                *(float4 *)&S[(lane & 3) * 1024 + cl] = make_float4(v[0], v[1], v[2], v[3]);
+                acc = (v4f){0.f, 0.f, 0.f, 0.f};
+            }
+        };
+        CIn cA = fetch_c(0), cB = fetch_c(T > 1 ? 1 : 0);
+#pragma unroll 1
+        for (int t = 0; t < T; t += 2) {
+            step(cA, t);
+            step(cB, t + 1);
+        }
+        __syncthreads();
+        if (myq < nq) {
+            const int cend = min(1024, kc - cb);
+            if (cb == 0) {
+                u64 mn = KEY_MAX;
+                for (int c = 0; c < cend; c += 64) {
+                    const int cc = c + lane;
+                    const u64 key = ((u64)ordered_bits(S[wv * 1024 + c + lane]) << 32) | (u32)cc;
+                    mn = (cc < kc && key < mn) ? key : mn;
+                }
+                const u64 bnd = readlane64(wave_sort64(mn, lane), Ksel - 1);
+                sel.init(bnd == KEY_MAX ? KEY_MAX : bnd + 1ull, nullptr, 64, Ksel);
+            }
+            for (int c = 0; c < cend; c += 64) {
+                const int cc = cb + c + lane;
+                const u64 key = ((u64)ordered_bits(S[wv * 1024 + c + lane]) << 32) | (u32)cc;
+                sel.push(cc < kc && key < sel.thr(), key, Ksel, lane);
+            }
+        }
+    }
+    if (myq >= nq) return;
+    const int cnt = sel.finish(Ksel, lane);
+    const WSel<true> ex = refine_probes(sel, cnt, P, myq, cn.rf, lane);
+    const int fc = ex.finish(P, lane);
+    if (lane < fc) {
+        cn.out_list[(size_t)myq * P + lane] = (int)(u32)ex.top;
+        cn.out_dc[(size_t)myq * P + lane] = __uint_as_float((u32)(ex.top >> 32));
+    }
+}
+
 template <int M, int DS, int PG>
-__global__ __launch_bounds__(256) void qscan_coarse_kernel(const QScanArgs a, const CoarseNext cn)
+__global__ __launch_bounds__(256, 4) void qscan_coarse_kernel(const QScanArgs a, const CoarseNext cn)
 {
     extern __shared__ __attribute__((aligned(16))) unsigned char smem_raw[];
     if ((int)blockIdx.x < a.nq) {
         qscan_body<M, DS, PG, true, false>(a, smem_raw, (int)blockIdx.x);
+    } else if (cn.probes) {
+        coarse_probe_tile(cn, a.ix.centroids, a.ix.kc, a.ix.d, (int)blockIdx.x - a.nq, smem_raw);
     } else {
         const int t = (int)blockIdx.x - a.nq;
         coarse_sgpr_tile<RIDER_QW>(cn.queries, a.ix.centroids, cn.out, cn.nq, a.ix.kc, a.ix.d, t % cn.ncx, t / cn.ncx, (float *)smem_raw);
diff --git a/ivfadc.jl_amd/index.py b/ivfadc.jl_amd/index.py
--- a/ivfadc.jl_amd/index.py
+++ b/ivfadc.jl_amd/index.py
@@ -370,6 +370,11 @@
         nat.check(nat.lib().ivfadc_set_next_queries(self._h, int(nq), C.c_void_p(d_queries_ptr) if d_queries_ptr else None,
                                                     C.c_uint64(int(token))))
 
+    def rider_info(self):
+        rf, ps = C.c_int(0), C.c_int(0)
+        nat.check(nat.lib().ivfadc_get_rider_info(self._h, C.byref(rf), C.byref(ps)))
+        return {"rider_form": rf.value, "probe_source": ps.value}
+
     def set_query_token(self, token):
         nat.check(nat.lib().ivfadc_set_query_token(self._h, C.c_uint64(int(token))))
 
```

Result: slower. 49.02 million (-1.5%).
